# aliddell/acquire-zarr

Hardware: AMD Instinct MI355X
Metric: input GB/s, device-resident multiscale downsample, uint16 frames @1/2/4/8 GPU (higher is better)
Workload: dtype u16

## Files before the change

acquire-zarr_amd/aqz/__init__.py:

```python
from __future__ import annotations

import ctypes as C
import os
import subprocess

import numpy as np

PKG_DIR = os.path.dirname(os.path.dirname(os.path.abspath(__file__)))
LIB_PATH = os.environ.get("AQZ_LIB") or os.path.join(PKG_DIR, "libaqz_gpu.so")

UINT8, UINT16, UINT32, UINT64, INT8, INT16, INT32, INT64, FLOAT32, FLOAT64 = range(10)
DECIMATE, MEAN, MIN, MAX = range(4)
SPACE, CHANNEL, TIME, OTHER = range(4)
MEM_HOST, MEM_DEVICE, MEM_HOST_PINNED = 0, 1, 2

NP_DTYPES = {UINT8: np.uint8, UINT16: np.uint16, UINT32: np.uint32,
             UINT64: np.uint64, INT8: np.int8, INT16: np.int16,
             INT32: np.int32, INT64: np.int64, FLOAT32: np.float32,
             FLOAT64: np.float64}

STATUS = {0: "Success", 1: "InvalidArgument", 2: "Overflow", 3: "InvalidIndex",
          4: "NotYetImplemented", 5: "InternalError", 6: "OutOfMemory",
          9: "InvalidSettings", 12: "WriteOutOfBounds"}

# ... 140 lines not shown
    build_library()
    _preload_hip_runtime()
    L = C.CDLL(LIB_PATH)
    vp, sz, i32, u32, u64 = C.c_void_p, C.c_size_t, C.c_int32, C.c_uint32, C.c_uint64
    D = C.POINTER(Dimension)
    sig = {
        "aqz_version": ([], C.c_char_p),
        "aqz_status_message": ([i32], C.c_char_p),
        "aqz_last_error": ([], C.c_char_p),
        "aqz_device_count": ([C.POINTER(i32)], i32),
        "aqz_dims_create": ([D, sz, i32, C.POINTER(sz), C.POINTER(vp)], i32),
        "aqz_dims_destroy": ([vp], None),
        "aqz_dims_ndims": ([vp], sz),
        "aqz_dims_get": ([vp, sz, D], i32),
        "aqz_dims_tile_group_offset": ([vp, u64], u32),
        "aqz_dims_chunk_internal_offset": ([vp, u64], u64),
        "aqz_dims_chunk_lattice_index": ([vp, u64, u32], u32),
        "aqz_dims_transpose_frame_id": ([vp, u64], u64),
        "aqz_dims_bytes_per_chunk": ([vp], u64),
        "aqz_dims_number_of_chunks_in_memory": ([vp], u32),
        "aqz_dims_frames_per_chunk_layer": ([vp], u64),
        "aqz_dims_shard_index_for_chunk": ([vp, u32], u32),
        "aqz_dims_shard_internal_index": ([vp, u32], u32),
        "aqz_dims_shard_geometry": ([vp, C.POINTER(u32), C.POINTER(u32), C.POINTER(u32)], i32),
        "aqz_dims_skipped_internal_indices": ([vp, u32, u32, C.POINTER(u32), sz,
                                               C.POINTER(sz)], i32),
        "aqz_pyramid_levels": ([D, sz, u32, C.POINTER(u32), D, sz], i32),
        "aqz_dims_split_frame_rows": ([vp, vp, u64, u32, u32, u32, vp, sz, vp, sz], i32),
        "aqz_stage_split_level0_host": ([vp, vp, u64, u64, u32, vp, sz, vp, sz], i32),
        "aqz_stage_split_level0_rows": ([vp, vp, u64, u32, u32, vp, u32, vp, sz, vp, sz], i32),
        "aqz_dims_dim1_banding": ([vp, C.POINTER(i32), C.POINTER(u32), C.POINTER(u64),
                                   C.POINTER(u32)], i32),
        "aqz_downsampling_method_name": ([i32], C.c_char_p),
        "aqz_downsampling_metadata_json": ([i32, C.c_char_p, sz, C.POINTER(sz)], i32),
        "aqz_downsampler_create": ([C.POINTER(ArrayDescC), C.POINTER(vp)], i32),
        "aqz_downsampler_destroy": ([vp], None),
        "aqz_downsampler_n_levels": ([vp], u32),
        "aqz_downsampler_level_dims": ([vp, u32, D, sz, C.POINTER(sz)], i32),
        "aqz_downsampler_add_frame": ([vp, vp, sz, i32], i32),
        "aqz_downsampler_take_frame": ([vp, u32, vp, sz, i32, C.POINTER(sz), C.POINTER(i32)], i32),
        "aqz_downsampler_method_name": ([vp], C.c_char_p),
        "aqz_downsampler_metadata_json": ([vp, C.c_char_p, sz, C.POINTER(sz)], i32),
        "aqz_stage_create": ([C.POINTER(ArrayDescC), C.POINTER(StageOptionsC), C.POINTER(vp)], i32),
        "aqz_stage_create_bench": ([C.POINTER(ArrayDescC), C.POINTER(StageOptionsC),
                                    C.POINTER(StageBenchOptionsC), C.POINTER(vp)], i32),
        "aqz_stage_wait_stream": ([vp, vp], i32),
        "aqz_stage_band_geometry": ([vp, u32, C.POINTER(i32), C.POINTER(u32), C.POINTER(u64),
                                     C.POINTER(u32)], i32),
        "aqz_stage_copy_band_async": ([vp, u32, u64, u32, vp, sz, vp, sz], i32),
        "aqz_stage_memory_usage": ([vp, C.POINTER(MemoryUsageC)], i32),
        "aqz_stage_estimate_memory": ([C.POINTER(ArrayDescC), C.POINTER(StageOptionsC),
                                       C.POINTER(MemoryUsageC)], i32),
        "aqz_stage_estimate_memory_bench": ([C.POINTER(ArrayDescC), C.POINTER(StageOptionsC),
                                             C.POINTER(StageBenchOptionsC),
                                             C.POINTER(MemoryUsageC)], i32),
        "aqz_stage_placement_report": ([vp, C.POINTER(PlacementReportC)], i32),
        "aqz_stage_destroy": ([vp], None),
        "aqz_stage_n_levels": ([vp], u32),
        "aqz_stage_level_dims": ([vp, u32, D, sz, C.POINTER(sz)], i32),
        "aqz_stage_level_layout": ([vp, u32, C.POINTER(LevelLayoutC)], i32),
        "aqz_stage_set_stream": ([vp, vp], i32),
        "aqz_stage_set_tuning": ([vp, u32, u32], i32),
        "aqz_stage_append": ([vp, vp, u64, i32], i32),
        "aqz_stage_synchronize": ([vp], i32),
        "aqz_stage_frames_written": ([vp, u32], u64),
        "aqz_stage_copy_layer": ([vp, u32, u64, vp, sz, vp, sz, i32], i32),
        "aqz_stage_copy_layer_async": ([vp, u32, u64, vp, sz, vp, sz], i32),
        "aqz_stage_frames_consumed": ([vp], u64),
        "aqz_stage_wait_consumed": ([vp, u64], i32),
        "aqz_stage_last_ticket": ([vp], u64),
        "aqz_stage_copies_completed": ([vp], u64),
        "aqz_stage_wait_ticket": ([vp, u64], i32),
        "aqz_stage_wait_copies": ([vp], i32),
        "aqz_host_alloc": ([sz, C.POINTER(vp)], i32),
        "aqz_host_free": ([vp], None),
        "aqz_stage_device_layer": ([vp, u32, u64, C.POINTER(vp), C.POINTER(vp)], i32),
        "aqz_stage_finalize": ([vp], i32),
        "aqz_stage_enable_kernel_timing": ([vp, i32], i32),
        "aqz_stage_kernel_timing": ([vp, C.POINTER(C.c_double), C.POINTER(u64)], i32),
        "aqz_stage_timing_mark": ([vp, i32], i32),
        "aqz_stage_timing_elapsed": ([vp, C.POINTER(C.c_double)], i32),
        "aqz_stage_dominant_kernel": ([vp], C.c_char_p),
        "aqz_stage_zstd_far_ranges": ([vp, u32], u32),
        "aqz_probe_hbm": ([i32, i32, u64, u32, C.POINTER(C.c_double), C.POINTER(u64)], i32),
        "aqz_stage_placement": ([vp, C.POINTER(C.c_double), sz, C.POINTER(sz),
                                 C.POINTER(u32)], i32),
        "aqz_stage_host_affinity": ([vp, C.POINTER(i32), C.POINTER(u32)], i32),
        "aqz_stage_compress_layer": ([vp, u32, u64, C.POINTER(CompressionC)], i32),
        "aqz_stage_compressed_offsets": ([vp, u32, u64, C.POINTER(u64), sz], i32),
        "aqz_stage_copy_compressed_async": ([vp, u32, u64, vp, sz], i32),
        "aqz_compressor_create": ([u64, u32, C.POINTER(CompressionC), C.POINTER(vp)], i32),
        "aqz_compressor_destroy": ([vp], None),
        "aqz_compressor_max_bytes": ([u64, u32], u64),
        "aqz_compressor_scratch_bytes": ([C.POINTER(CompressionC), u64, u32, u32], u64),
        "aqz_compressor_run": ([vp, vp, u64, u32, vp, sz, vp, vp], i32),
        "aqz_compressor_blocksize": ([vp], u32),
        "aqz_decompressor_create": ([u64, u32, C.POINTER(vp)], i32),
        "aqz_decompressor_create_for": ([u64, u32, u32, C.POINTER(vp)], i32),
        "aqz_decompressor_destroy": ([vp], None),
        "aqz_decompressor_scratch_bytes": ([u64, u32], u64),
        "aqz_decompressor_scratch_bytes_for": ([u64, u32, u32], u64),
        "aqz_decompressor_last_run_counts": ([vp, C.POINTER(DecodeCountsC)], i32),
        "aqz_stage_verify_prepare": ([vp, u32], i32),
        "aqz_decompressor_run": ([vp, vp, sz, vp, u32, vp, u64, u64, vp, vp], i32),
        "aqz_stage_verify_layer": ([vp, u32, u64, vp, sz], i32),
        "aqz_stage_verify_result": ([vp, u32, u64, C.POINTER(u32), C.POINTER(u32)], i32),
        "aqz_stage_bench_replace_rings": ([vp, u32], i32),
        "aqz_stage_bench_set_ring_offset": ([vp, u64], i32),
        "aqz_stage_bind_host_thread": ([vp], i32),
        "aqz_stage_import_frames": ([vp, vp, u32, u64, u32, u32], i32),
        "aqz_stage_compression_done": ([vp, u32, u64, C.POINTER(C.c_int32)], i32),
        "aqz_stage_compressed_entries": ([vp, u32, u64, C.POINTER(ChunkEntryC), sz], i32),
        "aqz_stage_shard_geometry": ([vp, u32, C.POINTER(u32), C.POINTER(u32),
                                      C.POINTER(u32)], i32),
        "aqz_shard_table_bytes": ([u32], sz),
        "aqz_shard_table": ([vp, vp, u32, vp, sz], i32),
        "aqz_crc32c": ([vp, sz], u32),
        "aqz_shard_table_parse": ([vp, sz, u32, vp, vp, C.POINTER(i32)], i32),
        "aqz_reader_create": ([C.POINTER(ReaderDescC), C.POINTER(vp)], i32),
        "aqz_reader_destroy": ([vp], None),
        "aqz_reader_device_bytes": ([C.POINTER(ReaderDescC)], u64),
        "aqz_reader_layout": ([vp, C.POINTER(LevelLayoutC)], i32),
        "aqz_reader_load_frames": ([vp, vp, sz, i32, vp, vp, u32, i32, vp], i32),
        "aqz_reader_load_chunks": ([vp, vp, u64, vp, u32, vp], i32),
        "aqz_reader_read_frames": ([vp, u32, u32, vp, u64, vp], i32),
        "aqz_reader_status": ([vp, vp, sz, C.POINTER(u32)], i32),
    }
    for name, (args, res) in sig.items():
        f = getattr(L, name)
        f.argtypes = args
        f.restype = res
    _lib = L
    return L


def _check(status: int, what: str) -> None:
    if status != 0:
        msg = lib().aqz_last_error()
        raise AqzError(status, what + (": " + msg.decode() if msg else ""))


PROBE_READ, PROBE_COPY, PROBE_COPY_THIRD, PROBE_READ_THIRD = 0, 1, 2, 3
PROBE_PLAIN_STORES = 0x100
PROBE_PIECES = 0x200
PROBE_DEEP = 0x400


def probe_hbm(shape: int, nbytes: int = 512 << 20, reps: int = 20, device: int = 0):
    ms, rd = C.c_double(0), C.c_uint64(0)
    _check(lib().aqz_probe_hbm(device, shape, nbytes, reps, C.byref(ms), C.byref(rd)),
           "aqz_probe_hbm")
    return ms.value, rd.value


def device_count() -> int:
    n = C.c_int32(0)
    _check(lib().aqz_device_count(C.byref(n)), "aqz_device_count")
    return n.value


def _dims_c(dims):
    arr = (Dimension * len(dims))()
    for i, d in enumerate(dims):
        arr[i] = Dimension(*d)
    return arr

# ... 51 lines not shown

    def frames_per_chunk_layer(self):
        return lib().aqz_dims_frames_per_chunk_layer(self.h)

    def shard_index_for_chunk(self, c):
        return lib().aqz_dims_shard_index_for_chunk(self.h, c)

    def shard_internal_index(self, c):
        return lib().aqz_dims_shard_internal_index(self.h, c)

    def shard_geometry(self):
        a, b, c = C.c_uint32(), C.c_uint32(), C.c_uint32()
        _check(lib().aqz_dims_shard_geometry(self.h, C.byref(a), C.byref(b), C.byref(c)),
               "aqz_dims_shard_geometry")
        return a.value, b.value, c.value

    def skipped_internal_indices(self, shard, layer):
        n = C.c_size_t(0)
        _check(lib().aqz_dims_skipped_internal_indices(self.h, shard, layer, None, 0,
                                                       C.byref(n)), "skipped_internal")
        out = (C.c_uint32 * max(1, n.value))()
        _check(lib().aqz_dims_skipped_internal_indices(self.h, shard, layer, out, n.value,
                                                       C.byref(n)), "skipped_internal")
        return list(out[:n.value])

    def split_frame_rows(self, frame, frame_id, dst, has_data, row_begin=0, row_end=None,
                         chunk0=0):
        frame = np.ascontiguousarray(frame)
        if row_end is None:
            row_end = frame.shape[-2] if frame.ndim >= 2 else 0
        assert dst.dtype == np.uint8 and has_data.dtype == np.uint8
        _check(lib().aqz_dims_split_frame_rows(self.h, frame.ctypes.data, frame_id, row_begin,
                                               row_end, chunk0, dst.ctypes.data, dst.nbytes,
                                               has_data.ctypes.data, has_data.size),
               "aqz_dims_split_frame_rows")

    def dim1_banding(self):
        a, b, c, d = C.c_int32(), C.c_uint32(), C.c_uint64(), C.c_uint32()
        _check(lib().aqz_dims_dim1_banding(self.h, C.byref(a), C.byref(b), C.byref(c),
                                           C.byref(d)), "aqz_dims_dim1_banding")
        return bool(a.value), b.value, c.value, d.value


def downsampling_method_name(method):
    return lib().aqz_downsampling_method_name(method).decode()


def downsampling_metadata_json(method):
    n = C.c_size_t(0)
    _check(lib().aqz_downsampling_metadata_json(method, None, 0, C.byref(n)), "metadata")
    buf = C.create_string_buffer(n.value + 1)
    _check(lib().aqz_downsampling_metadata_json(method, buf, n.value + 1, C.byref(n)),
           "metadata")
    return buf.value.decode()


def estimate_memory(dims, dtype, method, max_levels=0, layer_slots=0,
                    max_batch_frames=0, storage_order=None, placement_tries=0,
                    level0_split_on_host=False, **bench):
    d, keep = _desc(dims, dtype, method, max_levels, True, storage_order, 0)
    o = StageOptionsC(layer_slots, max_batch_frames, 0, 0, 0, placement_tries,
                      int(bool(level0_split_on_host)))
    m = MemoryUsageC()
    b = _bench_options(bench)
    if b is not None:
        _check(lib().aqz_stage_estimate_memory_bench(C.byref(d), C.byref(o), C.byref(b),
                                                     C.byref(m)),
               "aqz_stage_estimate_memory_bench")
    else:
        _check(lib().aqz_stage_estimate_memory(C.byref(d), C.byref(o), C.byref(m)),
               "aqz_stage_estimate_memory")
    return {"device_bytes": m.device_bytes, "pinned_bytes": m.pinned_bytes}


def compressor_max_bytes(chunk_bytes, n_chunks):
    return lib().aqz_compressor_max_bytes(chunk_bytes, n_chunks)


def compressor_scratch_bytes(codec, chunk_bytes, typesize, n_chunks):
    c = CompressionC(*codec)
    return lib().aqz_compressor_scratch_bytes(C.byref(c), chunk_bytes, typesize, n_chunks)


def pyramid_levels(dims, max_levels=0):
    d = _dims_c(dims)
    n = C.c_uint32(0)
    _check(lib().aqz_pyramid_levels(d, len(dims), max_levels, C.byref(n), None, 0),
           "aqz_pyramid_levels")
    nd = max(3, len(dims))
    out = (Dimension * (n.value * nd))()
    _check(lib().aqz_pyramid_levels(d, len(dims), max_levels, C.byref(n), out,
                                    n.value * nd), "aqz_pyramid_levels")
    return [_tuples(out[l * nd:(l + 1) * nd], nd) for l in range(n.value)]


def _desc(dims, dtype, method, max_levels, multiscale, storage_order, device):
    keep = [_dims_c(dims)]
    order = None
    if storage_order is not None:
        order = (C.c_size_t * len(storage_order))(*storage_order)
        keep.append(order)
    d = ArrayDescC(keep[0], len(dims), dtype, 1 if multiscale else 0, method,
                   max_levels, order, device)
    return d, keep


class HostBuffer:

    def __init__(self, nbytes):
        p = C.c_void_p()
        _check(lib().aqz_host_alloc(nbytes, C.byref(p)), "aqz_host_alloc")
        self.ptr = p.value
        self.nbytes = nbytes
        self.array = np.ctypeslib.as_array((C.c_uint8 * nbytes).from_address(self.ptr))

    def view(self, dtype=np.uint8, shape=None):
        a = self.array.view(dtype)
        return a.reshape(shape) if shape is not None else a

    def close(self):
        if getattr(self, "ptr", None) and _lib is not None:
            self.array = None
            _lib.aqz_host_free(self.ptr)
            self.ptr = None

    def __del__(self):
        self.close()


def _ptr(buf):
    if isinstance(buf, HostBuffer):
        return buf.ptr, MEM_HOST_PINNED
    if isinstance(buf, np.ndarray):
        assert buf.flags.c_contiguous
        return buf.ctypes.data, MEM_HOST
    if hasattr(buf, "data_ptr"):
        assert buf.is_contiguous()
        return buf.data_ptr(), (MEM_DEVICE if buf.is_cuda else MEM_HOST)
    raise TypeError(type(buf))


class Downsampler:

    def __init__(self, dims, dtype, method, max_levels=0, storage_order=None,
                 device=0):
        self.dtype = dtype
        d, self._keep = _desc(dims, dtype, method, max_levels, True,
                              storage_order, device)
        h = C.c_void_p()
        _check(lib().aqz_downsampler_create(C.byref(d), C.byref(h)),
               "aqz_downsampler_create")
        self.h = h

    def __del__(self):
        if getattr(self, "h", None) and _lib is not None:
            _lib.aqz_downsampler_destroy(self.h)
            self.h = None

    def n_levels(self):
        return lib().aqz_downsampler_n_levels(self.h)

    def level_dims(self, level):
        out = (Dimension * 16)()
        n = C.c_size_t(0)
        _check(lib().aqz_downsampler_level_dims(self.h, level, out, 16, C.byref(n)),
               "level_dims")
# ... 143 lines not shown
    def frames_written(self, level):
        return lib().aqz_stage_frames_written(self.h, level)

    def split_level0_host(self, frames_ptr, n_frames, first_frame, dst_ptr, cap, has_ptr,
                          has_cap, chunk0=0):
        _check(lib().aqz_stage_split_level0_host(self.h, frames_ptr, n_frames, first_frame,
                                                 chunk0, dst_ptr, cap, has_ptr, has_cap),
               "split_level0_host")

    def split_level0_rows(self, frame_ptr, frame_id, row_begin, row_end, dst_ptr, cap,
                          has_ptr, has_cap, chunk0=0, frame_copy_ptr=None):
        _check(lib().aqz_stage_split_level0_rows(self.h, frame_ptr, frame_id, row_begin,
                                                 row_end, frame_copy_ptr, chunk0, dst_ptr, cap,
                                                 has_ptr, has_cap), "split_level0_rows")

    def frames_consumed(self):
        return lib().aqz_stage_frames_consumed(self.h)

    def copy_layer(self, level, layer):
        lay = self.layout(level)
        nbytes = lay["bytes_per_chunk"] * lay["chunks_per_layer"]
        out = np.empty(nbytes, dtype=np.uint8)
        flags = np.empty(lay["chunks_per_layer"], dtype=np.uint8)
        _check(lib().aqz_stage_copy_layer(self.h, level, layer, out.ctypes.data,
                                          nbytes, flags.ctypes.data, flags.size,
                                          MEM_HOST), "copy_layer")
        return out, flags

    def device_layer(self, level, layer):
        chunks, flags = C.c_void_p(), C.c_void_p()
        _check(lib().aqz_stage_device_layer(self.h, level, layer, C.byref(chunks),
                                            C.byref(flags)), "device_layer")
        return chunks.value, flags.value, layer // self.layout(level)["layer_slots"] + 1

    def copy_layer_async(self, level, layer, dst_ptr, cap, has_data_ptr=None,
                         has_data_cap=0):
        _check(lib().aqz_stage_copy_layer_async(self.h, level, layer, dst_ptr, cap,
                                                has_data_ptr, has_data_cap),
               "copy_layer_async")

    def wait_consumed(self, frames):
        _check(lib().aqz_stage_wait_consumed(self.h, frames), "wait_consumed")
        self._release_consumed()

    def last_ticket(self):
        return lib().aqz_stage_last_ticket(self.h)

    def copies_completed(self):
        return lib().aqz_stage_copies_completed(self.h)

    def wait_ticket(self, ticket):
        _check(lib().aqz_stage_wait_ticket(self.h, ticket), "wait_ticket")

    def wait_copies(self):
        _check(lib().aqz_stage_wait_copies(self.h), "wait_copies")

    def finalize(self):
        _check(lib().aqz_stage_finalize(self.h), "finalize")
        self._release_consumed()

    def enable_kernel_timing(self, on=True):
        _check(lib().aqz_stage_enable_kernel_timing(self.h, 1 if on else 0), "timing")

    def kernel_timing(self):
        ms = C.c_double(0)
        n = C.c_uint64(0)
        _check(lib().aqz_stage_kernel_timing(self.h, C.byref(ms), C.byref(n)), "timing")
        return ms.value, n.value

    def timing_mark(self, which):
        _check(lib().aqz_stage_timing_mark(self.h, which), "timing_mark")

    def timing_elapsed(self):
        ms = C.c_double(0)
        _check(lib().aqz_stage_timing_elapsed(self.h, C.byref(ms)), "timing_elapsed")
        return ms.value

    def dominant_kernel(self):
        return lib().aqz_stage_dominant_kernel(self.h).decode()

    def zstd_far_ranges(self, level):
        return lib().aqz_stage_zstd_far_ranges(self.h, level)

    def bind_host_thread(self):
        _check(lib().aqz_stage_bind_host_thread(self.h), "bind_host_thread")

    def host_affinity(self):
        node, n = C.c_int32(-1), C.c_uint32(0)
        _check(lib().aqz_stage_host_affinity(self.h, C.byref(node), C.byref(n)),
               "host_affinity")
        return node.value, n.value

    def placement(self):
        r = PlacementReportC()
        _check(lib().aqz_stage_placement_report(self.h, C.byref(r)), "placement_report")
        return {"candidates_ms": [round(r.ms[i], 5) for i in range(min(32, r.n))],
                "kept": r.kept, "kept_ms_final": round(r.kept_ms_final, 5),
                "reps": r.reps, "mode": r.mode,
                "peak_device_bytes": r.peak_device_bytes,
                "probe_bus_gbs": round(r.probe_bus_gbs, 1),
                "expected_ms": round(r.expected_ms, 5), "alg_bytes": r.alg_bytes,
                "accepted": bool(r.accepted),
                "stop": {1: "accepted", 2: "every try ran", 3: "no expectation (probe too small)",
                         4: "out of memory"}.get(r.stop, "no search"),
                "candidates_probe_gbs": [round(r.probe_gbs[i], 1)
                                         for i in range(min(32, r.n))]}

    def compress_layer(self, level, layer, codec=CODEC_BLOSC_LZ4, clevel=5, shuffle=1):
        c = CompressionC(codec, clevel, shuffle)
        _check(lib().aqz_stage_compress_layer(self.h, level, layer, C.byref(c)),
               "compress_layer")

    def compression_done(self, level, layer):
        d = C.c_int32(0)
        _check(lib().aqz_stage_compression_done(self.h, level, layer, C.byref(d)),
               "compression_done")
        return bool(d.value)

    def compressed_offsets(self, level, layer):
        n = self.layout(level)["chunks_per_layer"] + 1
        off = np.empty(n, dtype=np.uint64)
        _check(lib().aqz_stage_compressed_offsets(
            self.h, level, layer, off.ctypes.data_as(C.POINTER(C.c_uint64)), n),
            "compressed_offsets")
        return off

    def copy_compressed_async(self, level, layer, dst_ptr, cap):
        _check(lib().aqz_stage_copy_compressed_async(self.h, level, layer, dst_ptr, cap),
               "copy_compressed_async")

    def compressed_entries(self, level, layer):
        n = self.layout(level)["chunks_per_layer"]
        arr = (ChunkEntryC * n)()
        _check(lib().aqz_stage_compressed_entries(self.h, level, layer, arr, n),
               "compressed_entries")
        return [(e.chunk, e.shard, e.internal, e.offset, e.nbytes) for e in arr]

    def shard_geometry(self, level):
        a, b, c = C.c_uint32(), C.c_uint32(), C.c_uint32()
        _check(lib().aqz_stage_shard_geometry(self.h, level, C.byref(a), C.byref(b),
                                              C.byref(c)), "shard_geometry")
        return a.value, b.value, c.value

    def copy_compressed(self, level, layer):
        off = self.compressed_offsets(level, layer)
        out = np.empty(max(1, int(off[-1])), dtype=np.uint8)
        self.copy_compressed_async(level, layer, out.ctypes.data, out.nbytes)
        self.wait_copies()
        return out[:int(off[-1])], off

    def verify_prepare(self, codecs):
        _check(lib().aqz_stage_verify_prepare(self.h, codecs), "verify_prepare")

    def verify_layer(self, level, layer, frames_ptr=None, frames_bytes=0):
        _check(lib().aqz_stage_verify_layer(self.h, level, layer, frames_ptr, frames_bytes),
               "verify_layer")
        n, first = C.c_uint32(), C.c_uint32()
        _check(lib().aqz_stage_verify_result(self.h, level, layer, C.byref(n),
                                             C.byref(first)), "verify_result")
        return n.value, first.value


class Compressor:

    def __init__(self, chunk_bytes, typesize, codec=CODEC_BLOSC_LZ4, clevel=5, shuffle=1):
        c = CompressionC(codec, clevel, shuffle)
# ... 213 lines not shown
```

acquire-zarr_amd/csrc/aqz_capi.cpp:

```cpp
#include "aqz_gpu.h"
#include "aqz_gpu_bench.h"

#include "aqz_engine.hh"
#include "aqz_reader.hh"

#include <cstring>
#include <new>
#include <string>

using namespace aqz;

struct aqz_dims
{
    std::unique_ptr<ArrayDimensions> ad;
};
struct aqz_downsampler
{
    std::unique_ptr<GpuDownsampler> ds;
    int32_t sticky = AQZ_STATUS_SUCCESS;
};
struct aqz_stage
{
    std::unique_ptr<Stage> st;
    int32_t sticky = AQZ_STATUS_SUCCESS;
// ... 885 lines not shown
{
    return guard_sticky(
      st, [&] { st->st->device_layer(level, layer, chunks, has_data); });
}

aqz_status
aqz_stage_finalize(aqz_stage* st)
{
    return guard_sticky(st, [&] { st->st->finalize(); });
}

aqz_status
aqz_stage_split_level0_host(aqz_stage* st, const void* frames, uint64_t n_frames,
                            uint64_t first_frame, uint32_t chunk0, void* dst, size_t cap,
                            uint8_t* has_data, size_t has_data_cap)
{
    if (!st || !st->st)
        return AQZ_STATUS_INVALID_ARGUMENT;
    return guard([&] {
        st->st->split_level0_host(frames, n_frames, first_frame, chunk0, dst, cap, has_data,
                                  has_data_cap);
    });
}

aqz_status
aqz_stage_split_level0_rows(const aqz_stage* st, const void* frame, uint64_t frame_id,
                            uint32_t row_begin, uint32_t row_end, void* frame_copy,
                            uint32_t chunk0, void* dst, size_t cap, uint8_t* has_data,
                            size_t has_data_cap)
{
    if (!st || !st->st)
        return AQZ_STATUS_INVALID_ARGUMENT;
    return guard([&] {
        st->st->split_level0_rows(frame, frame_id, row_begin, row_end, frame_copy, chunk0, dst,
                                  cap, has_data, has_data_cap);
    });
}

aqz_status
aqz_stage_enable_kernel_timing(aqz_stage* st, int32_t enable)
{
    return guard_sticky(st, [&] { st->st->enable_timing(enable != 0); });
}

aqz_status
aqz_stage_kernel_timing(aqz_stage* st, double* total_ms, uint64_t* launches)
{
    return guard_sticky(st, [&] { st->st->timing(total_ms, launches); });
}

aqz_status
aqz_stage_timing_mark(aqz_stage* st, int32_t which)
{
    return guard_sticky(st, [&] { st->st->mark(which); });
}

aqz_status
aqz_stage_timing_elapsed(aqz_stage* st, double* ms)
{
    return guard_sticky(st, [&] {
        const double v = st->st->marked_ms();
        if (ms)
            *ms = v;
    });
}

const char*
aqz_stage_dominant_kernel(const aqz_stage* st)
{
    return st ? st->st->dominant_kernel() : "";
}

uint32_t
aqz_stage_zstd_far_ranges(const aqz_stage* st, uint32_t level)
{
    try {
        return st && st->st ? st->st->zstd_far_ranges(level) : 0;
    } catch (...) {
        return 0;
    }
}

aqz_status
aqz_stage_host_affinity(const aqz_stage* st, int32_t* numa_node, uint32_t* n_cpus)
{
    if (!st)
        return AQZ_STATUS_INVALID_ARGUMENT;
    if (numa_node)
        *numa_node = st->st->numa_node();
    if (n_cpus)
        *n_cpus = uint32_t(st->st->numa_cpus());
    return AQZ_STATUS_SUCCESS;
}

aqz_status
aqz_stage_placement_report(const aqz_stage* st, aqz_placement_report* out)
{
    if (!st || !out)
        return AQZ_STATUS_INVALID_ARGUMENT;
    const PlacementReport& r = st->st->placement();
    *out = aqz_placement_report{};
    out->n = uint32_t(r.ms.size());
    out->kept = uint32_t(r.kept);
    out->reps = r.reps;
    out->mode = r.mode;
    for (size_t i = 0; i < r.ms.size() && i < 32; ++i)
        out->ms[i] = r.ms[i];
    out->kept_ms_final = r.kept_ms_final;
    out->peak_device_bytes = r.peak_device;
    out->probe_bus_gbs = r.probe_bus_gbs;
    out->expected_ms = r.expected_ms;
    out->alg_bytes = r.alg_bytes;
    out->accepted = r.accepted ? 1u : 0u;
    out->stop = r.stop;
    for (size_t i = 0; i < r.probe_gbs.size() && i < 32; ++i)
        out->probe_gbs[i] = r.probe_gbs[i];
    return AQZ_STATUS_SUCCESS;
}

aqz_status
aqz_stage_placement(const aqz_stage* st, double* ms, size_t cap, size_t* n, uint32_t* kept)
{
    if (!st)
        return AQZ_STATUS_INVALID_ARGUMENT;
    const auto& v = st->st->placement_ms();
    if (n)
        *n = v.size();
    if (kept)
        *kept = uint32_t(st->st->placement_best());
    for (size_t i = 0; ms && i < v.size() && i < cap; ++i)
        ms[i] = v[i];
    return AQZ_STATUS_SUCCESS;
}

}

static Compression
to_compression(const aqz_compression* c)
{
    Compression k;
    k.codec = c->codec;
    k.clevel = c->clevel;
    k.shuffle = c->shuffle;
    return k;
}

aqz_status
aqz_stage_compress_layer(aqz_stage* st, uint32_t level, uint64_t layer,
                         const aqz_compression* comp)
{
    if (!comp)
        return AQZ_STATUS_INVALID_ARGUMENT;
    return guard_sticky(
      st, [&] { st->st->compress_layer(level, layer, to_compression(comp)); });
}

aqz_status
aqz_stage_compressed_offsets(aqz_stage* st, uint32_t level, uint64_t layer,
                             uint64_t* offsets, size_t n)
{
    if (!offsets)
        return AQZ_STATUS_INVALID_ARGUMENT;
    return guard_sticky(
      st, [&] { st->st->compressed_offsets(level, layer, offsets, n); });
}

aqz_status
aqz_stage_copy_compressed_async(aqz_stage* st, uint32_t level, uint64_t layer,
                                void* dst, size_t cap)
{
    if (!dst)
        return AQZ_STATUS_INVALID_ARGUMENT;
    return guard_sticky(
      st, [&] { st->st->copy_compressed_async(level, layer, dst, cap); });
}

aqz_status
aqz_compressor_create(uint64_t chunk_bytes, uint32_t typesize,
                      const aqz_compression* comp, aqz_compressor** out)
{
    if (!comp || !out)
        return AQZ_STATUS_INVALID_ARGUMENT;
    *out = nullptr;
    return guard([&] {
        auto h = std::make_unique<aqz_compressor>();
        h->c = std::make_unique<Compressor>(chunk_bytes, typesize, to_compression(comp));
        *out = h.release();
    });
}

void
aqz_compressor_destroy(aqz_compressor* c)
{
    delete c;
}

uint64_t
aqz_compressor_max_bytes(uint64_t chunk_bytes, uint32_t n_chunks)
{
    return Compressor::max_bytes(chunk_bytes, n_chunks);
}

uint64_t
aqz_compressor_scratch_bytes(const aqz_compression* comp, uint64_t chunk_bytes,
                             uint32_t typesize, uint32_t n_chunks)
{
    if (!comp)
        return 0;
    uint64_t n = 0;
    const aqz_status s = guard([&] {
        const Compression c = to_compression(comp);
        Compressor check(chunk_bytes, typesize, c);
        n = Compressor::scratch_bytes(c, chunk_bytes, typesize, n_chunks);
    });
    return s == AQZ_STATUS_SUCCESS ? n : 0;
}

uint32_t
aqz_compressor_blocksize(const aqz_compressor* c)
{
    return c && c->c ? c->c->blocksize() : 0;
}

aqz_status
aqz_compressor_run(aqz_compressor* c, const void* chunks, uint64_t pitch,
                   uint32_t n_chunks, void* dst, size_t dst_cap, uint64_t* offsets,
                   void* stream)
{
    if (!c || !chunks || !dst || !offsets)
        return AQZ_STATUS_INVALID_ARGUMENT;
    return guard_sticky(c, [&] {
        const uint64_t nb = c->c->chunk_bytes();
        if (pitch < nb)
            throw Error(1, "chunk pitch below the chunk size");
        if (dst_cap < Compressor::max_bytes(nb, n_chunks))
            throw Error(2, "destination below aqz_compressor_max_bytes");
        c->c->run(static_cast<const uint8_t*>(chunks), pitch, n_chunks, nullptr, 0,
                  static_cast<uint8_t*>(dst), offsets, static_cast<hipStream_t>(stream));
    });
}

static_assert(AQZ_DECODE_OK == dec::kOk && AQZ_DECODE_SKIPPED == dec::kSkipped &&
                AQZ_DECODE_BAD_HEADER == dec::kBadHeader &&
                AQZ_DECODE_CORRUPT == dec::kCorrupt &&
                AQZ_DECODE_UNSUPPORTED == dec::kUnsupported,
              "decode status values");

aqz_status
aqz_decompressor_create(uint64_t max_chunk_bytes, uint32_t max_chunks, aqz_decompressor** out)
{
    if (!out)
        return AQZ_STATUS_INVALID_ARGUMENT;
    *out = nullptr;
    return guard([&] {
        auto h = std::make_unique<aqz_decompressor>();
        h->d = std::make_unique<Decompressor>(max_chunk_bytes, max_chunks);
        *out = h.release();
    });
}

static_assert(AQZ_DECODE_CODEC_LZ4 == dec::kFamilyLz4 && AQZ_DECODE_CODEC_ZSTD == dec::kFamilyZstd &&
                AQZ_DECODE_ZSTD_PARALLEL == kDecodeZstdParallel,
              "decode codec bits");

aqz_status
aqz_decompressor_create_for(uint64_t max_chunk_bytes, uint32_t max_chunks, uint32_t codecs,
                            aqz_decompressor** out)
{
    if (!out)
        return AQZ_STATUS_INVALID_ARGUMENT;
    *out = nullptr;
    if (!decode_codecs_valid(codecs))
        return AQZ_STATUS_INVALID_ARGUMENT;
    return guard([&] {
        auto h = std::make_unique<aqz_decompressor>();
        h->d = std::make_unique<Decompressor>(max_chunk_bytes, max_chunks, true, codecs);
        *out = h.release();
    });
}

void
aqz_decompressor_destroy(aqz_decompressor* d)
{
    delete d;
}

uint64_t
aqz_decompressor_scratch_bytes(uint64_t max_chunk_bytes, uint32_t max_chunks)
{
    return Decompressor::scratch_bytes(max_chunk_bytes, max_chunks);
}

uint64_t
aqz_decompressor_scratch_bytes_for(uint64_t max_chunk_bytes, uint32_t max_chunks, uint32_t codecs)
{
    return Decompressor::scratch_bytes(max_chunk_bytes, max_chunks, true, codecs);
}

aqz_status
aqz_decompressor_last_run_counts(aqz_decompressor* d, aqz_decode_counts* out)
// ... 223 lines not shown
```

acquire-zarr_amd/csrc/aqz_codec.hh:

```
#pragma once

#include "aqz_zstd.hh"

#include <hip/hip_runtime.h>

#include <cstdint>

namespace aqz {

constexpr uint32_t kLz4StreamMax = 4096;
constexpr int kLz4HashLog = 10;

struct BloscGeom
{
    uint32_t nbytes;
    uint32_t typesize;
    uint32_t shuffle;
    uint32_t blocksize;
    uint32_t nfull;
    uint32_t left;
    uint32_t ns_full;
    uint32_t spc;
    uint32_t slot;
    uint32_t nblocks;
// ... 79 lines not shown
};

struct ZstdParams
{
    const uint8_t* src;
    uint64_t src_pitch;
    const uint8_t* chunks;
    uint64_t pitch;
    uint32_t n_chunks, nbytes, typesize, shuffle;
    uint32_t blosc;
    uint32_t seg_bytes;
    uint32_t nseg;
    uint32_t bps;
    uint32_t store_only;
    uint32_t match;
    uint32_t match_bits;
    uint32_t phist;
    uint32_t ngrp;
    uint32_t hgrp_log2;
    uint32_t fit;
    uint32_t* far;
    uint32_t far_tb;
    uint32_t far_slices;
    uint32_t far_log;
    uint32_t far_ranges;
    uint32_t far_warm;
    uint32_t dbg;
    const uint32_t* flags;
    uint32_t tag;
    const zstd::SeqTables* seqt;
    uint8_t* lits;
    uint64_t* seqs;
    uint32_t* snseq, *snlit, *stail;
    uint32_t* sval;
    uint32_t* hist;
    uint8_t* bkind;
    uint8_t* bltype;
    uint32_t* bpay;
    uint32_t* bseqb;
    uint32_t* bnlit;
    uint32_t* bpos;
    uint8_t* scratch;
    uint32_t* bnseq;
    ZstdSegTable* tab;
    uint32_t* carrier;
    uint32_t* scount;
    ZstdSeqSeg* sqt;
    uint32_t* scarrier;
    uint32_t* ssize;
    uint8_t* sraw;
    uint32_t* spos;
    uint32_t* fsize;
    uint8_t* mode;
    const uint32_t* order;
    uint64_t* offsets;
    uint64_t* cstart;
    uint8_t* out;
};

constexpr uint32_t kZSub = 4096;
constexpr uint32_t kZSubBlocks = zstd::kBlock / kZSub;
constexpr uint32_t kZSubSeq = 1024;
constexpr uint32_t kZHist1 = 12 * 1024;
constexpr uint32_t kZHist2 = 28 * 1024;
constexpr uint32_t kFarLog = 15;
constexpr uint32_t kFarMin = 5;
constexpr uint32_t kFarWarm = 256;
constexpr uint32_t kZOffMax = (1u << 24) - 4;
inline uint32_t
zstd_far_tag_bits(uint32_t seg_bytes, uint32_t slices, uint32_t far_log = kFarLog)
{
    uint32_t pb = 0, sb = 0;
    while (pb < 32 && (uint64_t(1) << pb) <= seg_bytes)
        ++pb;
    while ((1u << sb) < slices)
        ++sb;
    const uint32_t room = 32 - sb - far_log;
    const uint32_t tb = 32 - pb < room ? 32 - pb : room;
    return tb >= 6 ? tb : 0;
}

hipError_t launch_zstd(const ZstdParams& p, hipStream_t stream);

}
```

acquire-zarr_amd/csrc/aqz_codec.hip:

```cpp
#include "aqz_codec.hh"
#include "aqz_zstd.hh"

namespace aqz {

BloscGeom
make_blosc_geom(uint32_t nbytes, uint32_t typesize, uint32_t shuffle)
{
    BloscGeom g{};
    g.nbytes = nbytes;
    g.typesize = typesize;
    g.shuffle = shuffle;
    uint64_t bs = uint64_t(kLz4StreamMax) * typesize;
    if (bs > nbytes)
        bs = nbytes;
    bs -= bs % typesize;
    if (bs == 0)
        bs = nbytes;
    g.blocksize = uint32_t(bs);
    g.nfull = bs ? nbytes / g.blocksize : 0;
    g.left = bs ? nbytes % g.blocksize : 0;
    g.ns_full = (typesize <= 16 && g.blocksize / typesize >= 128) ? typesize : 1;
    g.spc = g.nfull * g.ns_full + (g.left ? 1u : 0u);
    g.nblocks = g.nfull + (g.left ? 1u : 0u);
    g.slot = g.blocksize / g.ns_full;
// ... 2057 lines not shown
        const uint8_t* scr = p.scratch + uint64_t(g) * zstd::kBlock;
        const uint32_t ns = p.bnseq[g];
        const ZstdSeqSeg& Q = p.sqt[z.seg];
        const bool fitted = ns > 0 && Q.mode == 2;
        const bool scar = fitted && p.scarrier[z.seg] == z.b;
        const uint32_t sd = scar ? Q.desc_n : 0;
        uint8_t* q = d + 3;
        uint32_t lit_bytes = pay;
        if (p.bltype[g] == 2) {
            const ZstdSegTable& T = p.tab[z.grp];
            const bool carry = p.carrier[z.grp] == z.b;
            const uint32_t cs = pay + (carry ? T.tree_n : 0);
            const uint32_t lh = zstd::lit_header_huf_bytes(nl, cs);
            if (t == 0) {
                zstd::write_block_header(d, last, 2, lh + cs + sq + sd);
                zstd::write_lit_header_huf(d + 3, carry ? 2 : 3, nl, cs);
            }
            q += lh;
            if (carry) {
                for (uint32_t i = t; i < T.tree_n; i += 256)
                    q[i] = T.tree[i];
                q += T.tree_n;
            }
        } else {
            const uint32_t lh = zstd::lit_header_raw_bytes(nl);
            if (t == 0) {
                zstd::write_block_header(d, last, 2, lh + nl + sq + sd);
                zstd::write_lit_header_raw(d + 3, 0, nl);
            }
            q += lh;
            lit_bytes = nl;
        }
        if (!fitted) {
            copy_bytes(q, scr, lit_bytes + sq);
        } else {
            const uint32_t kc = ns < 128 ? 1u : ns < 0x7F00 ? 2u : 3u;
            copy_bytes(q, scr, lit_bytes + kc);
            if (t == 0)
                q[lit_bytes + kc] = scar ? uint8_t(2u << 6 | 2u << 4 | 2u << 2)
                                         : uint8_t(3u << 6 | 3u << 4 | 3u << 2);
            uint8_t* qd = q + lit_bytes + kc + 1;
            for (uint32_t i = t; i < sd; i += 256)
                qd[i] = Q.desc[i];
            copy_bytes(qd + sd, scr + lit_bytes + kc + 1, sq - kc - 1);
        }
    }
}

}

hipError_t
launch_shuffle_blocks(const ShuffleParams& p, hipStream_t stream)
{
    if (p.n_chunks == 0 || p.nblocks == 0)
        return hipSuccess;
    if (p.nblocks > 0x7fffffffu || p.n_chunks > 65535u)
        return hipErrorInvalidValue;
    const uint64_t wg = uint64_t(p.nblocks) * p.n_chunks;
    const uint32_t parts = uint32_t(std::min<uint64_t>(16, std::max<uint64_t>(1, (2048 + wg - 1) / wg)));
    hipLaunchKernelGGL(shuffle_blocks, dim3(p.nblocks, p.n_chunks, parts), dim3(256), 0, stream,
                       p);
    return hipGetLastError();
}

hipError_t
launch_blosc_lz4(const BloscParams& p, hipStream_t stream)
{
    if (p.n_chunks == 0)
        return hipSuccess;
    const uint64_t ns = uint64_t(p.n_chunks) * p.g.spc;
    if (ns > 0x7fffffffull || p.g.spc == 0)
        return hipErrorInvalidValue;
    hipLaunchKernelGGL(lz4_streams, dim3(uint32_t(ns)), dim3(64), 0, stream, p);
    hipLaunchKernelGGL(chunk_layout, dim3(p.n_chunks), dim3(256), 0, stream, p);
    hipLaunchKernelGGL(scan_offsets, dim3(1), dim3(256), 0, stream, p.fsize, p.order,
                       p.offsets, p.cstart, p.n_chunks);
    hipLaunchKernelGGL(write_frames, dim3(uint32_t(ns)), dim3(256), 0, stream, p);
    return hipGetLastError();
}

hipError_t
launch_zstd(const ZstdParams& p, hipStream_t stream)
{
    if (p.n_chunks == 0)
        return hipSuccess;
    const uint64_t nseg = uint64_t(p.n_chunks) * p.nseg;
    const uint64_t nblk = nseg * p.bps;
    if (nblk * kZSubBlocks > 0x7fffffffull || p.nseg == 0 || p.bps == 0 ||
        uint64_t(p.bps) * zstd::kBlock < p.seg_bytes)
        return hipErrorInvalidValue;
    if (p.hgrp_log2 > 5 || p.ngrp != ((p.bps + (1u << p.hgrp_log2) - 1) >> p.hgrp_log2))
        return hipErrorInvalidValue;
    if (!p.store_only) {
        hipError_t e = hipMemsetAsync(p.scount, 0, nseg * 192 * 4, stream);
        if (e != hipSuccess)
            return e;
        if (p.match) {
            e = hipMemsetAsync(p.hist, 0, nblk * 256 * 4, stream);
            if (e != hipSuccess)
                return e;
            const dim3 gd(uint32_t(nblk * kZSubBlocks));
            if (p.far) {
                const uint32_t S = p.far_slices;
                if (!(S == 1 || S == 2 || S == 4 || S == 8) || p.far_tb < 6 ||
                    p.far_log < 10 || p.far_log > kFarLog ||
                    p.far_tb + p.far_log + (S == 8 ? 3 : S == 4 ? 2 : S == 2 ? 1 : 0) > 32 ||
                    (reinterpret_cast<uintptr_t>(p.src) & 3u) || (p.src_pitch & 3u) ||
                    (p.seg_bytes & 3u))
                    return hipErrorInvalidValue;
                static const hipError_t attr = hipFuncSetAttribute(
                  reinterpret_cast<const void*>(zstd_far),
                  hipFuncAttributeMaxDynamicSharedMemorySize, int(4u << kFarLog));
                if (attr != hipSuccess)
                    return attr;
                const uint32_t R = p.far_ranges;
                if (!(R == 1 || R == 2 || R == 4 || R == 8))
                    return hipErrorInvalidValue;
                hipLaunchKernelGGL(zstd_far, dim3(uint32_t(nseg * p.far_slices * R)),
                                   dim3(kFarThreads), size_t(4) << p.far_log, stream, p);
            }
            if (p.phist == 0 && !p.far)
                hipLaunchKernelGGL((zstd_parse<0, kLz4HashLog>), gd, dim3(64), 0, stream, p);
            else if (p.phist <= kZHist1 && !p.far)
                hipLaunchKernelGGL((zstd_parse<kZHist1, 13>), gd, dim3(64), 0, stream, p);
            else if (!p.far)
                hipLaunchKernelGGL((zstd_parse<kZHist2, 14>), gd, dim3(64), 0, stream, p);
            else if (p.phist == 0)
                hipLaunchKernelGGL((zstd_parse<0, kLz4HashLog, true>), gd, dim3(64), 0, stream, p);
            else if (p.phist <= kZHist1)
                hipLaunchKernelGGL((zstd_parse<kZHist1, 13, true>), gd, dim3(64), 0, stream, p);
            else
                hipLaunchKernelGGL((zstd_parse<kZHist2, 14, true>), gd, dim3(64), 0, stream, p);
        } else {
            hipLaunchKernelGGL(zstd_hist, dim3(uint32_t(nblk)), dim3(256), 0, stream, p);
        }
        hipLaunchKernelGGL(zstd_table, dim3(uint32_t(nseg * p.ngrp)), dim3(64), 0, stream, p);
        hipLaunchKernelGGL(zstd_encode, dim3(uint32_t(nblk)), dim3(256), 0, stream, p);
        hipLaunchKernelGGL(zstd_seqtab, dim3(uint32_t(nseg)), dim3(64), 0, stream, p);
        if (p.match)
            hipLaunchKernelGGL(zstd_seqenc, dim3(uint32_t(nseg * ((p.bps + 63) / 64))), dim3(64), 0,
                               stream, p);
        hipLaunchKernelGGL(zstd_segment, dim3(uint32_t(nseg)), dim3(64), 0, stream, p);
    }
    hipLaunchKernelGGL(zstd_chunk, dim3(p.n_chunks), dim3(256), 0, stream, p);
    hipLaunchKernelGGL(scan_offsets, dim3(1), dim3(256), 0, stream, p.fsize, p.order,
                       p.offsets, p.cstart, p.n_chunks);
    hipLaunchKernelGGL(zstd_write, dim3(uint32_t(nblk)), dim3(256), 0, stream, p);
    return hipGetLastError();
}

}
```

acquire-zarr_amd/csrc/aqz_engine.cpp:

```cpp
#include <cstdio>
#include "aqz_engine.hh"

#include <hsa/hsa_ext_amd.h>
#include "aqz_zstd.hh"

#include <algorithm>
#include <atomic>
#include <cstdlib>
#include <cstring>
#include <thread>

namespace aqz {


constexpr int kMemDevice = 1;
constexpr int kMemHostPinned = 2;

void
hip_check(hipError_t e, const char* what)
{
    if (e != hipSuccess) {
        (void)hipGetLastError();
        throw Error(e == hipErrorOutOfMemory ? 6 : 5,
                    std::string(what) + ": " + hipGetErrorString(e));
// ... 199 lines not shown
    const uint64_t per = std::max<uint64_t>(1, copy_piece_bytes() / bpc);
    for (uint64_t c = 0; c < n; c += per) {
        const uint64_t m = std::min<uint64_t>(per, n - c);
        if (m > 1)
            hip_check(hipMemcpy2DAsync(static_cast<uint8_t*>(dst) + c * bpc, bpc,
                                       src + c * pitch, pitch, bpc, m, kind, stream),
                      "hipMemcpy2DAsync");
        else
            memcpy_pieces(static_cast<uint8_t*>(dst) + c * bpc, src + c * pitch, bpc,
                          kind, stream);
    }
}

static unsigned
copy_workers()
{
    if (const char* s = std::getenv("AQZ_COPY_THREADS"))
        return unsigned(std::max(0, std::atoi(s)));
    const unsigned hw = std::max(1u, std::thread::hardware_concurrency());
    return std::min(7u, hw / 2);
}

static hipMemcpyKind
kind_from(int src_mem, int dst_mem)
{
    if (src_mem == kMemDevice)
        return dst_mem == kMemDevice ? hipMemcpyDeviceToDevice
                                     : hipMemcpyDeviceToHost;
    return dst_mem == kMemDevice ? hipMemcpyHostToDevice : hipMemcpyHostToHost;
}

static bool
method_valid(int32_t m)
{
    return m >= 0 && m < 4;
}

static bool
pinned_host(const void* p)
{
    hipPointerAttribute_t a{};
    if (hipPointerGetAttributes(&a, p) != hipSuccess) {
        (void)hipGetLastError();
        return false;
    }
    return a.type == hipMemoryTypeHost;
}

static bool
find_hsa_agents(int device, hsa_agent_t* gpu, hsa_agent_t* cpu)
{
    hipDeviceProp_t prop{};
    if (hipGetDeviceProperties(&prop, device) != hipSuccess || hsa_init() != HSA_STATUS_SUCCESS)
        return false;
    struct Find
    {
        uint32_t bdf, domain;
        hsa_agent_t gpu{ 0 }, cpu{ 0 };
    } f{ (uint32_t(prop.pciBusID) << 8) | (uint32_t(prop.pciDeviceID) << 3),
         uint32_t(prop.pciDomainID) };
    auto cb = [](hsa_agent_t a, void* data) -> hsa_status_t {
        auto* f = static_cast<Find*>(data);
        hsa_device_type_t t;
        if (hsa_agent_get_info(a, HSA_AGENT_INFO_DEVICE, &t) != HSA_STATUS_SUCCESS)
            return HSA_STATUS_SUCCESS;
        if (t == HSA_DEVICE_TYPE_CPU && !f->cpu.handle)
            f->cpu = a;
        if (t == HSA_DEVICE_TYPE_GPU) {
            uint32_t bdf = 0, dom = 0;
            hsa_agent_get_info(a, hsa_agent_info_t(HSA_AMD_AGENT_INFO_BDFID), &bdf);
            hsa_agent_get_info(a, hsa_agent_info_t(HSA_AMD_AGENT_INFO_DOMAIN), &dom);
            if ((bdf & ~7u) == f->bdf && dom == f->domain)
                f->gpu = a;
        }
        return HSA_STATUS_SUCCESS;
    };
    if (hsa_iterate_agents(cb, &f) != HSA_STATUS_SUCCESS || !f.gpu.handle || !f.cpu.handle)
        return false;
    *gpu = f.gpu;
    *cpu = f.cpu;
    return true;
}

Stage::Stage(const ArrayDesc& desc, const StageOptions& opt)
  : desc_(desc)
  , opt_(opt)
{
    bpp_ = bytes_of_type(desc.dtype);
    if (desc.multiscale && !method_valid(desc.method))
        throw Error(1, "Invalid downsampling method");
    if (opt_.layer_slots == 0)
        opt_.layer_slots = 2;
    if (opt_.max_batch_frames == 0)
        opt_.max_batch_frames = 64;
    if (opt_.level0_on_host)
        opt_.skip_level0_split = true;

    auto base = std::make_unique<ArrayDimensions>(desc.dims, desc.dtype,
                                                  desc.storage_order);
    if (base->needs_xy_transposition()) {
        if (opt_.level0_on_host)
            throw Error(9, "level0_split_on_host needs storage rows = acquisition rows "
                           "(no XY-transposed storage order)");
        xy_ = true;
        const size_t nd = desc.dims.size();
        acq_rows_ = desc.dims[nd - 2].array_size_px;
        acq_cols_ = desc.dims[nd - 1].array_size_px;
    }
    std::vector<std::vector<Dim>> levels;
    if (desc.multiscale)
        levels = make_pyramid_levels(base->dims(), desc.max_levels,
                                     opt_.force_levels);
    else
        levels = { base->dims() };

    hip_check(hipSetDevice(desc.device), "hipSetDevice");
    hip_check(hipStreamCreateWithFlags(&own_stream_, hipStreamNonBlocking),
              "hipStreamCreate");
    stream_ = own_stream_;
    {
        const char* e = std::getenv("AQZ_NUMA");
        char bus[64] = { 0 };
        if (!(e && std::atoi(e) == 0) &&
            hipDeviceGetPCIBusId(bus, int(sizeof(bus)), desc.device) == hipSuccess)
            numa_cpus_ = numa_cpus_for_pci(bus, &numa_node_);
        (void)hipGetLastError();
    }

    const size_t n = base->ndims();
    const uint32_t B = opt_.max_batch_frames;
    DevBuf spacer;
    if (opt_.ring_spacer)
        spacer.alloc(opt_.ring_spacer, opt_.ring_malloc_flags);
    lv_.resize(levels.size());
    for (size_t k = 0; k < levels.size(); ++k) {
        StageLevel& L = lv_[k];
        L.dims = levels[k];
        if (k == 0)
            L.ad = std::move(base);
        else
            L.ad = std::make_unique<ArrayDimensions>(L.dims, desc.dtype);
        L.W = L.dims[n - 1].array_size_px;
        L.H = L.dims[n - 2].array_size_px;
        L.planes = L.dims[n - 3].array_size_px;
        if (k > 0)
            L.xy_shrinks = L.W < lv_[k - 1].W || L.H < lv_[k - 1].H;
        L.tw = L.dims[n - 1].chunk_size_px;
        L.th = L.dims[n - 2].chunk_size_px;
        L.ntx = parts_along(L.W, L.tw);
        L.nty = parts_along(L.H, L.th);
        L.bpc = L.ad->bytes_per_chunk();
        L.n_chunks = L.ad->number_of_chunks_in_memory();
        const uint64_t F = L.ad->frames_per_chunk_layer();
        if (F == 0 || F > 0x7fffffffull)
            throw Error(9, "unsupported frames per chunk layer");
        L.F = uint32_t(F);
        L.pitch = L.bpc + opt_.chunk_pad;
        L.slot_bytes = L.pitch * L.n_chunks;
        L.layer_bytes = L.bpc * L.n_chunks;
        L.n_slots = std::max<uint32_t>(opt_.layer_slots,
                                       (B - 1 + L.F - 1) / L.F + 1);
        L.slot_layer.assign(L.n_slots, -1);

        L.h_tab_off.resize(L.F);
        L.h_tab_grp.resize(L.F);
        for (uint32_t fl = 0; fl < L.F; ++fl) {
// ... 65 lines not shown
        }
    }
    {
        uint32_t tz = 0;
        while (tz < 6 && ((lv_[0].th >> tz) & 1u) == 0)
            ++tz;
        const uint32_t nf = fused_3d_ ? n_levels() - 1 : n_fused_;
        rh_log2_ = std::max<uint32_t>(std::max<uint32_t>(4, nf), tz);
        if (fused_3d_) {
            const uint32_t RW = uint32_t(512 / bpp_);
            fused_3d_ = lv_[0].W % RW == 0 && (lv_[0].H % (1u << rh_log2_)) == 0 &&
                        lv_[0].th % (1u << rh_log2_) == 0 &&
                        lv_[0].tw % uint32_t(16 / bpp_) == 0 &&
                        (1u << rh_log2_) <= uint32_t(kMaxRegionRows);
        }
    }
    knobs_ = opt_.knobs;
    xcd_rot_ = opt_.xcd_rot;
    nt_mode_ = opt_.nt_mode & 7u;
    if (const uint32_t v = opt_.region_rows_log2) {
        if (v >= std::max<uint32_t>(4, n_fused_) && (1u << v) <= uint32_t(kMaxRegionRows))
            rh_log2_ = v;
    }
    if (xy_ && fused_2d_) {
        const bool tail = n_levels() - 1 > n_fused_;
        xy_direct_ = bpp_ <= 4 && rh_log2_ == 6 && !(knobs_ & 128u) &&
                     (!tail || n_fused_ >= 5) && !(knobs_ & 4096u) &&
                     (uint64_t(acq_cols_) * bpp_) % 16 == 0;
    } else if (xy_ && fused_3d_) {
        xy_direct_ = bpp_ <= 4 && rh_log2_ == 6 && n_levels() - 1 <= 4 &&
                     !(knobs_ & 256u) && !(knobs_ & 4096u) &&
                     (uint64_t(acq_cols_) * bpp_) % 16 == 0;
    }

    const Dim& d0 = lv_[0].dims[0];
    if (d0.array_size_px > 0) {
        max_frames_ = 1;
        for (size_t i = 0; i + 2 < n; ++i)
            max_frames_ *= lv_[0].dims[i].array_size_px;
    }
    if (opt_.z_slab_begin != 0 || opt_.z_slab_end != 0) {
        const uint64_t p0 = lv_[0].planes;
        const uint64_t b0 = opt_.z_slab_begin, e0 = opt_.z_slab_end;
        if (n < 4 || p0 == 0 || b0 >= e0 || e0 > p0)
            throw Error(1, "z slab needs a z dimension and 0 <= begin < end <= planes");
        if (opt_.first_frame % p0 != 0)
            throw Error(1, "with a z slab, first_frame must start a z stack");
        slab_len_ = e0 - b0;
        for (auto& L : lv_) {
            const uint64_t pk = L.planes;
            if ((b0 * pk) % p0 != 0 || (e0 * pk) % p0 != 0)
                throw Error(9, "z slab does not align with the z pyramid");
            slab_skip_.push_back(pk - (e0 - b0) * pk / p0);
        }
        opt_.first_frame += b0;
    }
    if (opt_.first_frame > 0) {
        const uint64_t p0 = std::max<uint32_t>(1, lv_[0].planes);
        for (auto& L : lv_) {
            const uint64_t pk = std::max<uint32_t>(1, L.planes);
            if ((opt_.first_frame * pk) % p0 != 0)
                throw Error(9, "first_frame does not align with the z pyramid");
            L.frames_written = opt_.first_frame * pk / p0;
            L.level_frame_count = uint32_t(L.frames_written);
        }
    }
    pend_.resize(lv_.size());
    for (int j = 0; j < 2; ++j) {
        hip_check(hipEventCreateWithFlags(&h2d_ev_[j], hipEventDisableTiming),
                  "hipEventCreate");
        hip_check(hipEventCreateWithFlags(&consume_ev_[j], hipEventDisableTiming),
                  "hipEventCreate");
    }
    {
        int least = 0, greatest = 0;
        hip_check(hipDeviceGetStreamPriorityRange(&least, &greatest),
                  "hipDeviceGetStreamPriorityRange");
        hip_check(hipStreamCreateWithPriority(&h2d_, hipStreamNonBlocking, greatest),
                  "hipStreamCreate");
        hip_check(hipStreamCreateWithPriority(&d2h_, hipStreamNonBlocking, greatest),
                  "hipStreamCreate");
        for (hipStream_t* cs : { &comp_, &comp_lo_ })
            hip_check(hipStreamCreateWithFlags(cs, hipStreamNonBlocking), "hipStreamCreate");
        hip_check(hipStreamCreateWithPriority(&comp_lo2_, hipStreamNonBlocking, least),
                  "hipStreamCreate");
    }
    if (const char* e = std::getenv("AQZ_D2H_SDMA"); e && std::atoi(e) != 0)
        sdma_d2h_ = find_hsa_agents(desc.device, &hsa_gpu_, &hsa_cpu_);
    for (auto& L : lv_) {
        hip_check(hipEventCreateWithFlags(&L.ops_ev, hipEventDisableTiming),
                  "hipEventCreate");
        if (!L.ring.p)
            continue;
        L.ready_ev.assign(L.n_slots, nullptr);
        L.copy_ev.assign(L.n_slots, nullptr);
        L.copy_pending.assign(L.n_slots, 0);
        for (uint32_t s = 0; s < L.n_slots; ++s) {
            hip_check(hipEventCreateWithFlags(&L.ready_ev[s], hipEventDisableTiming),
                      "hipEventCreate");
            hip_check(hipEventCreateWithFlags(&L.copy_ev[s], hipEventDisableTiming),
                      "hipEventCreate");
        }
        L.flag_bytes.alloc(size_t(L.n_slots) * L.n_chunks);
    }

    calibrate_placement();
    hip_check(hipStreamSynchronize(stream_), "hipStreamSynchronize");
}

void
Stage::place_level(StageLevel& L, uint8_t* at)
{
    if (at)
        L.ring.set_view(at, L.slot_bytes * L.n_slots);
    else
        L.ring.alloc(L.slot_bytes * L.n_slots, opt_.ring_malloc_flags & ~kRingsPlain);
    L.flags.alloc(size_t(L.n_chunks) * L.n_slots * 4);
    hip_check(hipMemsetAsync(L.ring.p, 0, L.ring.n, stream_), "hipMemsetAsync");
    hip_check(hipMemsetAsync(L.flags.p, 0, L.flags.n, stream_), "hipMemsetAsync");
    std::vector<FrameRef> tab(L.period);
    for (uint64_t fid = 0; fid < L.period; ++fid) {
        const uint64_t slot = fid / L.F;
        tab[fid].tiles = L.ring.p + slot * L.slot_bytes + L.h_tab_off[fid % L.F];
        tab[fid].flags = reinterpret_cast<uint32_t*>(L.flags.p) + slot * L.n_chunks +
                         L.h_tab_grp[fid % L.F];
    }
    L.ref_table.alloc(size_t(L.period) * sizeof(FrameRef));
    hip_check(hipMemcpy(L.ref_table.p, tab.data(), size_t(L.period) * sizeof(FrameRef),
                        hipMemcpyHostToDevice),
              "hipMemcpy");
}

void
Stage::calibrate_placement()
{
    const uint32_t tries = opt_.placement_tries;
    const uint32_t reps = std::max<uint32_t>(1, opt_.placement_reps);
    uint64_t ring_bytes = 0, set_bytes = 0;
    std::vector<bool> has_ring(lv_.size());
    for (size_t k = 0; k < lv_.size(); ++k) {
        has_ring[k] = lv_[k].ring.p != nullptr;
        ring_bytes += lv_[k].ring.n;
        set_bytes += lv_[k].ring.n + lv_[k].flags.n + lv_[k].ref_table.n;
    }
    uint32_t n = opt_.max_batch_frames;
    if (fused_3d_ && !fused_2d_)
        n = n / g3d_ * g3d_;
    if (tries <= 1 || n == 0 || !(fused_2d_ || fused_3d_) || (xy_ && !xy_direct_) ||
        ring_bytes < (uint64_t(256) << 20))
        return;
    const bool arena = arena_.p != nullptr;
    if (arena)
        set_bytes = set_bytes - ring_bytes + arena_.physical();
    const uint64_t fb0 = uint64_t(lv_[0].W) * lv_[0].H * bpp_;
    DevBuf src;
    alloc_large(src, size_t(n) * fb0, arena);
    hip_check(hipMemsetAsync(src.p, 0, src.n, stream_), "hipMemsetAsync");
    hip_check(launch_fill_random(src.p, src.n, 0x5eedull, stream_), "fill launch");
    uint64_t live = memory_usage().device + src.n;
    uint64_t peak = live;
    hipEvent_t a = nullptr, b = nullptr;
    hip_check(hipEventCreate(&a), "hipEventCreate");
    hip_check(hipEventCreate(&b), "hipEventCreate");
    std::vector<uint64_t> fw0, lfc0;
    for (const auto& L : lv_) {
        fw0.push_back(L.frames_written);
        lfc0.push_back(L.level_frame_count);
    }
    constexpr uint32_t kWarm = 2;
    std::vector<uint64_t> emitted(lv_.size(), 0);
    auto restore = [&]() {
        for (size_t k = 0; k < lv_.size(); ++k) {
            lv_[k].frames_written = fw0[k];
            lv_[k].level_frame_count = uint32_t(lfc0[k]);
            lv_[k].slot_layer.assign(lv_[k].n_slots, -1);
        }
    };
    auto elapsed = [&]() {
        hip_check(hipEventSynchronize(b), "hipEventSynchronize");
// ... 127 lines not shown
        lv_[k].ring = std::move(best.ring[k]);
        lv_[k].flags = std::move(best.flags[k]);
        lv_[k].ref_table = std::move(best.ref[k]);
    }
    rep.kept_ms_final = measure();
    rep.peak_device = peak;
    placement_ = rep;
    for (auto& L : lv_) {
        if (!L.ring.p)
            continue;
        hip_check(hipMemsetAsync(L.ring.p, 0, L.ring.n, stream_), "hipMemsetAsync");
        hip_check(hipMemsetAsync(L.flags.p, 0, L.flags.n, stream_), "hipMemsetAsync");
    }
    hip_check(hipStreamSynchronize(stream_), "hipStreamSynchronize");
    (void)hipEventDestroy(a);
    (void)hipEventDestroy(b);
}

void
Stage::grant_access(int device)
{
    if (!arena_.p || !arena_.vmm_span)
        return;
    std::lock_guard<std::mutex> lk(access_mu_);
    if (std::find(granted_.begin(), granted_.end(), device) != granted_.end())
        return;
    hipMemAccessDesc acc{};
    acc.location.type = hipMemLocationTypeDevice;
    acc.location.id = device;
    acc.flags = hipMemAccessFlagsProtReadWrite;
    hip_check(hipMemSetAccess(arena_.p, arena_.vmm_span, &acc, 1), "hipMemSetAccess");
    granted_.push_back(device);
}

void
Stage::place_rings_at(uint64_t offset)
{
    uint64_t at = offset;
    for (size_t k = 0; k < lv_.size(); ++k) {
        StageLevel& L = lv_[k];
        if (!(k == 0 && opt_.skip_level0_split)) {
            place_level(L, arena_.p + at);
            at += (L.slot_bytes * L.n_slots + 0xffffull) & ~0xffffull;
        }
    }
}

void
Stage::set_ring_offset(uint64_t offset)
{
    if (!arena_.p)
        throw Error(1, "the stage has no ring arena (bench option ring_arena_bytes)");
    if (offset % 256 || offset + arena_rings_ > arena_.n)
        throw Error(1, "ring offset outside the arena's slack (or not 256-B aligned)");
    hip_check(hipStreamSynchronize(stream_), "hipStreamSynchronize");
    place_rings_at(offset);
    for (auto& L : lv_) {
        L.frames_written = 0;
        L.level_frame_count = 0;
        L.slot_layer.assign(L.n_slots, -1);
    }
    hip_check(hipStreamSynchronize(stream_), "hipStreamSynchronize");
}

void
Stage::replace_rings(uint32_t mask)
{
    synchronize();
    for (size_t k = 0; k < lv_.size() && k < 32; ++k) {
        StageLevel& L = lv_[k];
        if (!((mask >> k) & 1u) || !L.ring.p)
            continue;
        held_.push_back(std::move(L.ring));
        held_.push_back(std::move(L.flags));
        held_.push_back(std::move(L.ref_table));
        place_level(L);
    }
    hip_check(hipStreamSynchronize(stream_), "hipStreamSynchronize");
}

Stage::~Stage()
{
    zpool_.reset();
    for (auto& L : lv_)
        for (auto& v : L.peer_ev)
            for (const auto& e : v)
                (void)hipEventSynchronize(e.get());
    if (stream_)
        (void)hipStreamSynchronize(stream_);
    for (hipStream_t s : { h2d_, comp_, comp_lo_, comp_lo2_, d2h_ })
        if (s) {
            (void)hipStreamSynchronize(s);
            (void)hipStreamDestroy(s);
        }
    for (int j = 0; j < 2; ++j)
        for (hipEvent_t e : { h2d_ev_[j], consume_ev_[j] })
            if (e)
                (void)hipEventDestroy(e);
    for (size_t i = inflight_head_; i < inflight_.size(); ++i)
        if (inflight_[i].first)
            free_ev_.push_back(inflight_[i].first);
    for (const Ticket& t : tickets_) {
        if (t.ev)
            free_ev_.push_back(t.ev);
        if (t.sig.handle) {
            while (hsa_signal_wait_scacquire(t.sig, HSA_SIGNAL_CONDITION_LT, 1, UINT64_MAX,
                                             HSA_WAIT_STATE_BLOCKED) > 0) {
            }
            free_sig_.push_back(t.sig);
        }
    }
    for (hipEvent_t e : free_ev_)
        (void)hipEventDestroy(e);
    for (hsa_signal_t g : free_sig_)
        (void)hsa_signal_destroy(g);
    for (auto& L : lv_) {
        if (L.ops_ev)
            (void)hipEventDestroy(L.ops_ev);
        for (hipEvent_t e : L.ready_ev)
            if (e)
                (void)hipEventDestroy(e);
        for (hipEvent_t e : L.copy_ev)
            if (e)
                (void)hipEventDestroy(e);
        for (hipEvent_t e : L.comp_ev)
            if (e)
                (void)hipEventDestroy(e);
        for (hipEvent_t e : L.cdone_ev)
            if (e)
                (void)hipEventDestroy(e);
        for (hipEvent_t e : L.zin_ev)
            if (e)
                (void)hipEventDestroy(e);
        for (hipEvent_t e : L.verify_ev)
            if (e)
                (void)hipEventDestroy(e);
    }

    for (auto& pr : ev_pairs_) {
        (void)hipEventDestroy(pr.first);
        (void)hipEventDestroy(pr.second);
    }
    for (hipEvent_t e : mark_ev_)
        if (e)
            (void)hipEventDestroy(e);
    if (ext_ev_)
        (void)hipEventDestroy(ext_ev_);
    if (own_stream_)
        (void)hipStreamDestroy(own_stream_);
}

const std::vector<Dim>&
Stage::level_dims(uint32_t level) const
{
    if (level >= lv_.size())
        throw Error(3, "level out of range");
    return lv_[level].dims;
}

LevelLayout
Stage::layout(uint32_t level) const
{
    if (level >= lv_.size())
        throw Error(3, "level out of range");
    const StageLevel& L = lv_[level];
    return LevelLayout{ L.bpc,   L.n_chunks,
                        L.n_slots, L.F,
                        uint64_t(L.W) * L.H * bpp_, L.W,
                        L.H,     L.pitch };
}

void
Stage::set_stream(hipStream_t s)
{
    hip_check(hipStreamSynchronize(stream_), "hipStreamSynchronize");
    stream_ = s ? s : own_stream_;
}

uint64_t
Stage::frames_written(uint32_t level) const
{
    if (level >= lv_.size())
        throw Error(3, "level out of range");
    return lv_[level].frames_written;
}

void
Stage::synchronize()
{
    hip_check(hipStreamSynchronize(h2d_), "hipStreamSynchronize");
    hip_check(hipStreamSynchronize(stream_), "hipStreamSynchronize");
    hip_check(hipStreamSynchronize(comp_), "hipStreamSynchronize");
    hip_check(hipStreamSynchronize(comp_lo_), "hipStreamSynchronize");
    hip_check(hipStreamSynchronize(comp_lo2_), "hipStreamSynchronize");
    hip_check(hipStreamSynchronize(d2h_), "hipStreamSynchronize");
    retire_consumed(true);
}

void
Stage::note_consumed(hipStream_t s, uint64_t frames)
{
    appended_ += frames;
    if (!s) {
        if (inflight_head_ == inflight_.size())
            consumed_ = appended_;
        else
            inflight_.emplace_back(nullptr, appended_);
        return;
    }
    hipEvent_t e;
    if (free_ev_.empty()) {
        hip_check(hipEventCreateWithFlags(&e, hipEventDisableTiming), "hipEventCreate");
    } else {
        e = free_ev_.back();
        free_ev_.pop_back();
    }
    hip_check(hipEventRecord(e, s), "hipEventRecord");
    inflight_.emplace_back(e, appended_);
    retire_consumed(false);
}

void
Stage::retire_consumed(bool wait)
{
    while (inflight_head_ < inflight_.size()) {
        auto& [e, n] = inflight_[inflight_head_];
        if (e) {
            if (wait) {
                hip_check(hipEventSynchronize(e), "hipEventSynchronize");
            } else {
                const hipError_t q = hipEventQuery(e);
                if (q == hipErrorNotReady)
                    break;
                hip_check(q, "hipEventQuery");
            }
            free_ev_.push_back(e);
        }
        consumed_ = n;
        ++inflight_head_;
    }
    if (inflight_head_ == inflight_.size()) {
        inflight_.clear();
        inflight_head_ = 0;
    }
}

uint64_t
Stage::frames_consumed()
{
    retire_consumed(false);
    return consumed_;
}

void
Stage::wait_consumed(uint64_t frames)
{
    if (frames > appended_)
        throw Error(1, "wait_consumed beyond the frames appended");
    while (consumed_ < frames && inflight_head_ < inflight_.size()) {
        auto& [e, n] = inflight_[inflight_head_];
        if (e) {
            hip_check(hipEventSynchronize(e), "hipEventSynchronize");
            free_ev_.push_back(e);
        }
        consumed_ = n;
        ++inflight_head_;
    }
    retire_consumed(false);
}

uint64_t
Stage::issue_ticket()
{
    hipEvent_t e;
    if (free_ev_.empty()) {
        hip_check(hipEventCreateWithFlags(&e, hipEventDisableTiming), "hipEventCreate");
    } else {
        e = free_ev_.back();
        free_ev_.pop_back();
    }
    hip_check(hipEventRecord(e, d2h_), "hipEventRecord");
    tickets_.push_back(Ticket{ e, hsa_signal_t{ 0 } });
    ++tickets_issued_;
    (void)copies_completed();
    return tickets_issued_;
}

uint64_t
Stage::issue_ticket(hsa_signal_t sig)
{
    tickets_.push_back(Ticket{ nullptr, sig });
    ++tickets_issued_;
    (void)copies_completed();
    return tickets_issued_;
}

uint64_t
Stage::copies_completed(bool wait_all, uint64_t until)
{
    while (!tickets_.empty() && tickets_done_ < tickets_issued_) {
        const Ticket t = tickets_.front();
        const bool wait = wait_all || tickets_done_ < until;
        if (t.sig.handle) {
            if (wait) {
                while (hsa_signal_wait_scacquire(t.sig, HSA_SIGNAL_CONDITION_LT, 1, UINT64_MAX,
                                                 HSA_WAIT_STATE_BLOCKED) > 0) {
                }
            } else if (hsa_signal_load_scacquire(t.sig) > 0) {
                break;
            }
            free_sig_.push_back(t.sig);
        } else {
            if (wait) {
                hip_check(hipEventSynchronize(t.ev), "hipEventSynchronize");
            } else {
                const hipError_t q = hipEventQuery(t.ev);
                if (q == hipErrorNotReady)
                    break;
                hip_check(q, "hipEventQuery");
            }
            free_ev_.push_back(t.ev);
        }
        tickets_.pop_front();
        ++tickets_done_;
    }
    return tickets_done_;
}

void
Stage::wait_copies()
{
    hip_check(hipStreamSynchronize(comp_), "hipStreamSynchronize");
    hip_check(hipStreamSynchronize(comp_lo_), "hipStreamSynchronize");
    hip_check(hipStreamSynchronize(comp_lo2_), "hipStreamSynchronize");
    hip_check(hipStreamSynchronize(d2h_), "hipStreamSynchronize");
    (void)copies_completed(true);
}

void
Stage::append(const void* frames, uint64_t n_frames, int mem)
{
    if (n_frames == 0)
        return;
    if (!frames)
        throw Error(1, "null frames");
    finalized_ = false;
    const uint64_t fbytes = uint64_t(lv_[0].W) * lv_[0].H * bpp_;
    uint64_t n_ok = n_frames;
    if (max_frames_ > 0) {
        uint64_t room = max_frames_ - std::min(max_frames_, lv_[0].frames_written);
        if (slab_len_) {
            const uint64_t p0 = lv_[0].planes;
            const uint64_t stack = lv_[0].frames_written / p0;
            const uint64_t stacks = max_frames_ / p0;
            room = stack < stacks ? (stacks - stack) * slab_len_ - slab_done_ : 0;
        }
        n_ok = std::min(n_ok, room);
    }
    const auto* src = static_cast<const uint8_t*>(frames);
    const uint32_t B = opt_.max_batch_frames;
    for (uint64_t done = 0; done < n_ok;) {
        uint32_t b = uint32_t(std::min<uint64_t>(B, n_ok - done));
        if (slab_len_)
            b = uint32_t(std::min<uint64_t>(b, slab_len_ - slab_done_));
        const uint8_t* p = src + done * fbytes;
        if (mem == kMemDevice) {
            run_batch(p, b);
        } else {
            const int j = stage_idx_;
            stage_idx_ ^= 1;
            const size_t nbytes = size_t(b) * fbytes;
            alloc_large(d_stage_[j], size_t(B) * fbytes, opt_.codec.vmm);
            const uint8_t* hsrc = p;
            if (mem != kMemHostPinned) {
                h_stage_[j].alloc(size_t(B) * fbytes);
                hip_check(hipEventSynchronize(h2d_ev_[j]), "hipEventSynchronize");
                if (!pool_)
                    pool_ = std::make_unique<CopyPool>(copy_workers(), numa_cpus_);
                pool_->copy(h_stage_[j].p, p, nbytes);
                hsrc = h_stage_[j].p;
            }
            if (consume_rec_[j])
                hip_check(hipStreamWaitEvent(h2d_, consume_ev_[j], 0),
                          "hipStreamWaitEvent");
            memcpy_pieces(d_stage_[j].p, hsrc, nbytes, hipMemcpyHostToDevice, h2d_);
            hip_check(hipEventRecord(h2d_ev_[j], h2d_), "hipEventRecord");
            if (mem == kMemHostPinned)
                note_consumed(h2d_, b);
            hip_check(hipStreamWaitEvent(stream_, h2d_ev_[j], 0), "hipStreamWaitEvent");
            run_batch(d_stage_[j].p, b);
            hip_check(hipEventRecord(consume_ev_[j], stream_), "hipEventRecord");
            consume_rec_[j] = true;
        }
        if (mem == kMemDevice)
            note_consumed(stream_, b);
        else if (mem != kMemHostPinned)
            note_consumed(nullptr, b);
        done += b;
        if (slab_len_ && (slab_done_ += b) == slab_len_) {
            for (size_t k = 0; k < lv_.size(); ++k) {
                lv_[k].frames_written += slab_skip_[k];
                lv_[k].level_frame_count += uint32_t(slab_skip_[k]);
            }
            slab_done_ = 0;
        }
    }
    if (n_ok < n_frames)
        throw Error(12, "append beyond the array's bounded extent");
}

void
Stage::run_batch(const uint8_t* dsrc, uint32_t n)
{
    uint32_t n3 = 0;
    if (!fused_2d_ && fused_3d_) {
        bool idle = lv_[0].frames_written % g3d_ == 0 &&
                    reinterpret_cast<uintptr_t>(dsrc) % 16 == 0;
// ... 760 lines not shown
}

void
Stage::compressed_entries(uint32_t level, uint64_t layer, ChunkEntry* out, size_t n)
{
    if (level >= lv_.size())
        throw Error(3, "level out of range");
    StageLevel& L = lv_[level];
    const uint32_t slot = L.n_slots ? uint32_t(layer % L.n_slots) : 0;
    if (L.comp_layer.empty() || L.comp_layer[slot] != int64_t(layer))
        throw Error(3, "layer was not compressed (or its slot was reused)");
    if (n < L.n_chunks)
        throw Error(2, "entries too small");
    const uint64_t* off;
    if (L.comp_host[slot]) {
        HostLayerJob& j = *L.zjob[slot];
        j.wait();
        if (j.status)
            throw Error(j.status, "zstd compression failed");
        off = j.offsets.data();
    } else {
        hip_check(hipEventSynchronize(L.comp_ev[slot]), "hipEventSynchronize");
        off = reinterpret_cast<const uint64_t*>(L.h_coffsets[slot].p);
    }
    const uint32_t cl = uint32_t(layer % L.layers_per_shard);
    for (uint32_t i = 0; i < L.n_chunks; ++i) {
        const uint32_t c = L.h_order[i];
        out[i] = ChunkEntry{ c, L.h_shard[c], L.h_internal0[c] + cl * L.internal_stride, 0,
                             off[i], off[i + 1] - off[i] };
    }
}

void
Stage::shard_geometry(uint32_t level, uint32_t* chunks_per_shard, uint32_t* n_shards,
                      uint32_t* layers_per_shard) const
{
    if (level >= lv_.size())
        throw Error(3, "level out of range");
    const StageLevel& L = lv_[level];
    if (chunks_per_shard)
        *chunks_per_shard = L.chunks_per_shard;
    if (n_shards)
        *n_shards = L.n_shards;
    if (layers_per_shard)
        *layers_per_shard = L.layers_per_shard;
}

Compressor::Compressor(uint64_t chunk_bytes, uint32_t typesize, const Compression& c,
                       const CodecTuning& tune)
  : c_(c)
  , tune_(tune)
  , nbytes_(chunk_bytes)
  , typesize_(typesize)
{
    if (c.codec < 1 || c.codec > 3)
        throw Error(4, "unknown codec");
    if (c.codec != 3 && (c.shuffle < 0 || c.shuffle > 2 || c.clevel < 0 || c.clevel > 9))
        throw Error(1, "invalid compression settings");
    if (c.codec == 3 && (c.clevel < 0 || c.clevel > 22 || c.shuffle != 0))
        throw Error(1, "invalid zstd settings: level 0-22 and no shuffle");
    if (chunk_bytes == 0 || chunk_bytes > 0x7fffffefull || typesize == 0 ||
        typesize > 255)
        throw Error(1, "chunk size outside the blosc1 limits");
    if (c.codec == 1)
        g_ = make_blosc_geom(uint32_t(chunk_bytes), typesize, uint32_t(c.shuffle));
    store_only_ = c.codec != 3 && c.clevel == 0;
}

constexpr uint64_t kFarRangeCus = 256;

uint32_t
zstd_far_slices(const Compression& c, uint32_t typesize)
{
    (void)typesize;
    if (c.codec == 3) {
        const int zl = c.clevel == 0 ? 3 : c.clevel;
        return zl >= 7 ? 8u : zl >= 3 ? 4u : 0u;
    }
    if (c.codec == 2 && c.shuffle == 2 && c.clevel >= 2)
        return 1u;
    return 0u;
}

uint64_t
Compressor::scratch_bytes(const Compression& c, uint64_t chunk_bytes, uint32_t typesize,
                          uint32_t n_chunks)
{
    const uint64_t n = n_chunks;
    const bool store_only = c.codec != 3 && c.clevel == 0;
    uint64_t b = n * 4 + n + n * 8;
    if (c.codec == 1) {
        const BloscGeom g = make_blosc_geom(uint32_t(chunk_bytes), typesize, uint32_t(c.shuffle));
        const uint64_t ns = n * g.spc;
        return b + (store_only ? 1 : ns * g.slot) + ns * 8;
    }
    uint64_t seg = chunk_bytes, nseg1 = 1;
    if (c.codec == 2) {
        const ZstdBloscGeom g = make_zstd_blosc_geom(uint32_t(chunk_bytes), typesize);
        seg = g.blocksize;
        nseg1 = g.nblocks;
    }
    const uint64_t nseg = n * nseg1, bps = (seg + zstd::kBlock - 1) / zstd::kBlock;
    const uint32_t gl =
      zstd_huf_group_log2(c.codec == 2 ? uint32_t(c.shuffle) : 0u, typesize, uint32_t(seg),
                          c.clevel);
    const uint64_t nblk = nseg * bps, ngrp = nseg * ((bps + (1u << gl) - 1) >> gl);
    b += nseg * 4;
    if (c.codec == 2 && !store_only && (c.shuffle == 2 || (c.shuffle == 1 && typesize > 1)))
        b += n * chunk_bytes;
    if (store_only)
        return b;
    if (zstd_far_slices(c, typesize))
        b += nseg * seg * 4;
    const uint64_t nu = nblk * kZSubBlocks;
    b += nu * kZSub + nu * kZSubSeq * 8 + 4 * nu * 4;
    b += nblk * (1 + 4 + 4 + 4 + 256 * 4 + 1 + 4 + 4 + zstd::kBlock);
    b += nseg * (192 * 4 + sizeof(ZstdSeqSeg) + 4 + 1 + 4);
    b += ngrp * (sizeof(ZstdSegTable) + 4) + sizeof(zstd::SeqTables);
    return b;
}

void
Compressor::run(const uint8_t* chunks, uint64_t pitch, uint32_t n_chunks,
                const uint32_t* flags, uint32_t tag, uint8_t* out, uint64_t* offsets,
                hipStream_t stream, const uint32_t* order)
{
    if (c_.codec != 1) {
        run_zstd(chunks, pitch, n_chunks, flags, tag, out, offsets, stream, order);
        return;
    }
    const uint64_t ns = uint64_t(n_chunks) * g_.spc;
    alloc_large(scratch_, store_only_ ? 1 : ns * g_.slot, tune_.vmm);
    ssize_.alloc(ns * 4);
    spos_.alloc(ns * 4);
    fsize_.alloc(size_t(n_chunks) * 4);
    mode_.alloc(n_chunks);
    cstart_.alloc(size_t(n_chunks) * 8);
    BloscParams p{};
    p.g = g_;
    p.chunks = chunks;
    p.pitch = pitch;
    p.n_chunks = n_chunks;
    p.flags = flags;
    p.tag = tag;
    p.scratch = scratch_.p;
    p.ssize = reinterpret_cast<uint32_t*>(ssize_.p);
    p.spos = reinterpret_cast<uint32_t*>(spos_.p);
    p.fsize = reinterpret_cast<uint32_t*>(fsize_.p);
    p.mode = mode_.p;
    p.offsets = offsets;
    p.cstart = reinterpret_cast<uint64_t*>(cstart_.p);
    p.order = order;
    p.out = out;
    p.store_only = store_only_ ? 1 : 0;
    hip_check(launch_blosc_lz4(p, stream), "blosc-lz4 launch");
}

void
Compressor::run_zstd(const uint8_t* chunks, uint64_t pitch, uint32_t n_chunks,
                     const uint32_t* flags, uint32_t tag, uint8_t* out, uint64_t* offsets,
                     hipStream_t stream, const uint32_t* order)
{
    const bool blosc = c_.codec == 2;
    ZstdParams p{};
    p.chunks = chunks;
    p.pitch = pitch;
    p.n_chunks = n_chunks;
    p.nbytes = uint32_t(nbytes_);
    p.typesize = typesize_;
    p.shuffle = blosc ? uint32_t(c_.shuffle) : 0;
    p.blosc = blosc ? 1 : 0;
    p.store_only = store_only_ ? 1 : 0;
    p.flags = flags;
    p.tag = tag;
    if (blosc) {
        const ZstdBloscGeom g = make_zstd_blosc_geom(uint32_t(nbytes_), typesize_);
        p.seg_bytes = g.blocksize;
        p.nseg = g.nblocks;
    } else {
        p.seg_bytes = uint32_t(nbytes_);
        p.nseg = 1;
    }
    p.bps = (p.seg_bytes + zstd::kBlock - 1) / zstd::kBlock;
    p.hgrp_log2 = zstd_huf_group_log2(p.shuffle, typesize_, p.seg_bytes, c_.clevel);
    p.ngrp = (p.bps + (1u << p.hgrp_log2) - 1) >> p.hgrp_log2;
    p.phist = tune_.phist;
    p.match_bits = uint32_t(blosc ? zstd::kMatchBits : zstd::kMatchBitsFitted);
    p.fit = tune_.fit;
    p.src = chunks;
    p.src_pitch = pitch;
    p.dbg = tune_.parse & 15u;
    const bool shuffle = blosc && !store_only_ &&
                         (c_.shuffle == 2 || (c_.shuffle == 1 && typesize_ > 1));
    if (shuffle && n_chunks > 65535u)
        throw Error(1, "blosc-zstd with a shuffle takes at most 65535 chunks per run");
    if (shuffle) {
        alloc_large(zin_, size_t(n_chunks) * nbytes_, tune_.vmm);
        ShuffleParams sp{ chunks, pitch, n_chunks, flags, tag, p.nbytes, typesize_,
                          uint32_t(c_.shuffle), p.seg_bytes, p.nseg, zin_.p };
        hip_check(launch_shuffle_blocks(sp, stream), "shuffle launch");
        p.src = zin_.p;
        p.src_pitch = nbytes_;
    }
    const uint64_t nseg = uint64_t(n_chunks) * p.nseg, nblk = nseg * p.bps;
    p.match = tune_.match ? 1 : 0;
    if (!store_only_) {
        if (!seqt_.p) {
            zstd::SeqTables t;
            if (!zstd::build_seq_tables(t))
                throw Error(10, "zstd sequence tables");
            seqt_.alloc(sizeof(t));
            hip_check(hipMemcpy(seqt_.p, &t, sizeof(t), hipMemcpyHostToDevice), "hipMemcpy");
        }
        p.far_slices = zstd_far_slices(c_, typesize_);
        p.far_log = blosc ? 13u : kFarLog;
        p.far_tb = p.far_slices ? zstd_far_tag_bits(p.seg_bytes, p.far_slices, p.far_log) : 0;
        bool far = p.match && p.far_tb != 0 && (reinterpret_cast<uintptr_t>(p.src) & 3u) == 0 &&
                   (p.src_pitch & 3u) == 0 && (p.seg_bytes & 3u) == 0;
        far = far && tune_.far != 0;
        if (far) {
            alloc_large(far_, nseg * p.seg_bytes * 4, tune_.vmm);
            p.far = reinterpret_cast<uint32_t*>(far_.p);
            p.phist = 0;
            const uint64_t wgs = nseg * p.far_slices;
            const uint64_t steps = (uint64_t(p.seg_bytes) + kZSub - 1) / kZSub;
            const uint64_t cus = kFarRangeCus;
            const uint64_t warm = std::max<uint64_t>(kFarWarm, (2 * plane_bytes_ + kZSub - 1) / kZSub);
            p.far_warm = uint32_t(std::min<uint64_t>(warm, steps));
            p.far_ranges = 1;
            while (tune_.ranges && p.far_ranges < 8 && wgs * p.far_ranges * 2 <= cus &&
                   steps / (2u * p.far_ranges) >= warm)
                p.far_ranges *= 2;
        }
        far_ranges_ = far ? p.far_ranges : 0;
        if (p.match) {
            const uint64_t nu = nblk * kZSubBlocks;
            alloc_large(lits_, nu * kZSub, tune_.vmm);
            alloc_large(seqs_, nu * kZSubSeq * 8, tune_.vmm);
            snseq_.alloc(nu * 4);
            snlit_.alloc(nu * 4);
            stail_.alloc(nu * 4);
            sval_.alloc(nu * 4);
        }
        const uint64_t ngrp = nseg * p.ngrp;
        bltype_.alloc(nblk);
        bseqb_.alloc(nblk * 4);
        bnlit_.alloc(nblk * 4);
        bnseq_.alloc(nblk * 4);
        hist_.alloc(nblk * 256 * 4);
        scount_.alloc(nseg * 192 * 4);
        sqt_.alloc(nseg * sizeof(ZstdSeqSeg));
        scarrier_.alloc(nseg * 4);
        bkind_.alloc(nblk);
        bpay_.alloc(nblk * 4);
        bpos_.alloc(nblk * 4);
        alloc_large(scratch_, nblk * zstd::kBlock, tune_.vmm);
        tab_.alloc(ngrp * sizeof(ZstdSegTable));
        carrier_.alloc(ngrp * 4);
        sraw_.alloc(nseg);
        ssize_.alloc(nseg * 4);
    }
    spos_.alloc(nseg * 4);
    fsize_.alloc(size_t(n_chunks) * 4);
    mode_.alloc(n_chunks);
    cstart_.alloc(size_t(n_chunks) * 8);
    p.seqt = reinterpret_cast<const zstd::SeqTables*>(seqt_.p);
    p.lits = lits_.p;
    p.seqs = reinterpret_cast<uint64_t*>(seqs_.p);
    p.snseq = reinterpret_cast<uint32_t*>(snseq_.p);
    p.snlit = reinterpret_cast<uint32_t*>(snlit_.p);
    p.stail = reinterpret_cast<uint32_t*>(stail_.p);
    p.sval = reinterpret_cast<uint32_t*>(sval_.p);
    p.bltype = bltype_.p;
    p.bseqb = reinterpret_cast<uint32_t*>(bseqb_.p);
    p.bnlit = reinterpret_cast<uint32_t*>(bnlit_.p);
    p.hist = reinterpret_cast<uint32_t*>(hist_.p);
    p.bnseq = reinterpret_cast<uint32_t*>(bnseq_.p);
    p.scount = reinterpret_cast<uint32_t*>(scount_.p);
    p.sqt = reinterpret_cast<ZstdSeqSeg*>(sqt_.p);
    p.scarrier = reinterpret_cast<uint32_t*>(scarrier_.p);
    p.bkind = bkind_.p;
    p.bpay = reinterpret_cast<uint32_t*>(bpay_.p);
    p.bpos = reinterpret_cast<uint32_t*>(bpos_.p);
    p.scratch = scratch_.p;
    p.tab = reinterpret_cast<ZstdSegTable*>(tab_.p);
    p.carrier = reinterpret_cast<uint32_t*>(carrier_.p);
    p.ssize = reinterpret_cast<uint32_t*>(ssize_.p);
    p.sraw = sraw_.p;
    p.spos = reinterpret_cast<uint32_t*>(spos_.p);
    p.fsize = reinterpret_cast<uint32_t*>(fsize_.p);
    p.mode = mode_.p;
    p.order = order;
    p.offsets = offsets;
    p.cstart = reinterpret_cast<uint64_t*>(cstart_.p);
    p.out = out;
    hip_check(launch_zstd(p, stream), "zstd launch");
}

void
Stage::ensure_comp_slots(StageLevel& L)
{
    if (!L.cframes.empty())
        return;
    L.cframes.resize(L.n_slots);
    L.coffsets.resize(L.n_slots);
    L.h_coffsets.resize(L.n_slots);
    L.comp_ev.assign(L.n_slots, nullptr);
    L.cdone_ev.assign(L.n_slots, nullptr);
    L.cdone_pending.assign(L.n_slots, 0);
    L.cdone_ticket.assign(L.n_slots, 0);
    L.comp_layer.assign(L.n_slots, -1);
    L.comp_codec.assign(L.n_slots, 0);
    L.h_zin.resize(L.n_slots);
    L.h_zhas.resize(L.n_slots);
    L.zin_ev.assign(L.n_slots, nullptr);
    L.zjob.resize(L.n_slots);
    L.comp_host.assign(L.n_slots, 0);
    for (uint32_t s = 0; s < L.n_slots; ++s) {
        hip_check(hipEventCreateWithFlags(&L.comp_ev[s], hipEventDisableTiming),
                  "hipEventCreate");
        hip_check(hipEventCreateWithFlags(&L.cdone_ev[s], hipEventDisableTiming),
                  "hipEventCreate");
        hip_check(hipEventCreateWithFlags(&L.zin_ev[s], hipEventDisableTiming),
                  "hipEventCreate");
    }
}

static bool
zstd_on_host()
{
    const char* s = std::getenv("AQZ_ZSTD_HOST");
    return s && std::atoi(s) != 0;
}

static unsigned
zstd_workers()
{
    if (const char* s = std::getenv("AQZ_ZSTD_THREADS"))
        return unsigned(std::max(1, std::atoi(s)));
    const unsigned hw = std::max(1u, std::thread::hardware_concurrency());
    return std::min(16u, std::max(1u, hw - 1));
}

void
Stage::compress_layer_host(StageLevel& L, uint32_t slot, uint64_t layer,
                           const Compression& c)
{
    const hipStream_t cs = comp_stream(L);
    const ZstdLib& z = ZstdLib::get();
    if (!z.ok)
        throw Error(4, "libzstd.so.1 is not available: no zstd codecs");
    if (c.codec == 2 && (c.shuffle < 0 || c.shuffle > 2 || c.clevel < 0 || c.clevel > 9))
        throw Error(1, "invalid blosc compression settings");
    if (c.codec == 3 && (c.clevel < -131072 || c.clevel > z.max_clevel()))
        throw Error(1, "invalid zstd level");
    if (L.bpc > 0x7fffffefull)
        throw Error(1, "chunk size outside the blosc1 limits");
    ensure_comp_slots(L);
    if (!zpool_)
        zpool_ = std::make_unique<TaskPool>(zstd_workers(), numa_cpus_);
    if (L.zjob[slot])
        L.zjob[slot]->wait();
    else
        L.zjob[slot] = std::make_shared<HostLayerJob>();
    if (L.cdone_ticket[slot]) {
        (void)copies_completed(false, L.cdone_ticket[slot]);
        L.cdone_ticket[slot] = 0;
    }
    if (L.cdone_pending[slot]) {
        hip_check(hipStreamWaitEvent(cs, L.cdone_ev[slot], 0), "hipStreamWaitEvent");
        L.cdone_pending[slot] = 0;
    }
    L.h_zin[slot].alloc(L.layer_bytes);
    L.h_zhas[slot].alloc(L.n_chunks);
    hip_check(hipEventRecord(L.ready_ev[slot], stream_), "hipEventRecord");
    hip_check(hipStreamWaitEvent(cs, L.ready_ev[slot], 0), "hipStreamWaitEvent");
    const uint8_t* chunks = L.ring.p + slot * L.slot_bytes;
    const auto* flags = reinterpret_cast<const uint32_t*>(L.flags.p) + size_t(slot) * L.n_chunks;
    const uint32_t tag = uint32_t(layer / L.n_slots + 1);
    const bool shuffle = c.codec == 2 && (c.shuffle == 2 || (c.shuffle == 1 && bpp_ > 1));
    if (shuffle) {
        const ZstdBloscGeom g = make_zstd_blosc_geom(uint32_t(L.bpc), uint32_t(bpp_));
        L.d_zshuf.alloc(L.layer_bytes);
        ShuffleParams sp{ chunks, L.pitch, L.n_chunks, flags, tag, uint32_t(L.bpc),
                          uint32_t(bpp_), uint32_t(c.shuffle), g.blocksize, g.nblocks,
                          L.d_zshuf.p };
        hip_check(launch_shuffle_blocks(sp, cs), "shuffle launch");
        memcpy_pieces(L.h_zin[slot].p, L.d_zshuf.p, L.layer_bytes, hipMemcpyDeviceToHost,
                      cs);
    } else {
        copy_chunks(L.h_zin[slot].p, chunks, L.bpc, L.pitch, L.n_chunks,
                    hipMemcpyDeviceToHost, cs);
    }
    uint8_t* fb = L.flag_bytes.p + size_t(slot) * L.n_chunks;
    hip_check(launch_flags_to_bytes(flags, fb, L.n_chunks, tag, cs), "flags launch");
    hip_check(hipMemcpyAsync(L.h_zhas[slot].p, fb, L.n_chunks, hipMemcpyDeviceToHost, cs),
              "hipMemcpyAsync");
    hip_check(hipEventRecord(L.zin_ev[slot], cs), "hipEventRecord");
    hip_check(hipEventRecord(L.copy_ev[slot], cs), "hipEventRecord");
    L.copy_pending[slot] = 1;

    HostLayerJob& j = *L.zjob[slot];
    j.codec = c.codec;
    j.clevel = c.clevel;
    j.shuffle = c.codec == 2 ? c.shuffle : 0;
    j.typesize = uint32_t(bpp_);
    j.bpc = L.bpc;
    j.n_chunks = L.n_chunks;
    j.chunks = L.h_zin[slot].p;
    j.has_data = L.h_zhas[slot].p;
    j.order = L.h_order;
    const ZstdBloscGeom g = make_zstd_blosc_geom(uint32_t(L.bpc), uint32_t(bpp_));
    j.frame_cap = std::max<uint64_t>(z.compress_bound(L.bpc),
                                     L.bpc + 16 + 8ull * g.nblocks + 64);
    j.tmp.resize(size_t(j.frame_cap) * L.n_chunks);
    host_zstd_compress(*zpool_, L.zjob[slot],
                       [ev = L.zin_ev[slot]] { (void)hipEventSynchronize(ev); });
    L.comp_layer[slot] = int64_t(layer);
    L.comp_codec[slot] = c.codec;
    L.comp_host[slot] = 1;
}

void
Stage::compress_layer(uint32_t level, uint64_t layer, const Compression& c)
{
    if (level >= lv_.size())
        throw Error(3, "level out of range");
    StageLevel& L = lv_[level];
    const hipStream_t cs = comp_stream(L);
    if (!L.ring.p)
        throw Error(1, "level 0 is not split on the device by this stage");
    const uint32_t slot = uint32_t(layer % L.n_slots);
    if (L.slot_layer[slot] != int64_t(layer))
        throw Error(3, "chunk layer not resident");
    if ((c.codec == 2 || c.codec == 3) && zstd_on_host()) {
        compress_layer_host(L, slot, layer, c);
        return;
    }
    if (!L.comp || L.comp_cfg.codec != c.codec || L.comp_cfg.clevel != c.clevel ||
        L.comp_cfg.shuffle != c.shuffle) {
        hip_check(hipStreamSynchronize(cs), "hipStreamSynchronize");
        hip_check(hipStreamSynchronize(d2h_), "hipStreamSynchronize");
        L.comp = std::make_unique<Compressor>(L.bpc, uint32_t(bpp_), c, opt_.codec);
        L.comp->set_plane_bytes(uint64_t(L.tw) * L.th * bpp_);
        L.comp_cfg = c;
    }
    ensure_comp_slots(L);
    if (L.zjob[slot])
        L.zjob[slot]->wait();
    L.comp_host[slot] = 0;
    if (L.cdone_ticket[slot]) {
        (void)copies_completed(false, L.cdone_ticket[slot]);
        L.cdone_ticket[slot] = 0;
    }
    if (L.cdone_pending[slot]) {
        hip_check(hipStreamWaitEvent(cs, L.cdone_ev[slot], 0), "hipStreamWaitEvent");
        L.cdone_pending[slot] = 0;
    }
    const uint64_t cap = Compressor::max_bytes(L.bpc, L.n_chunks);
    if (L.cframes[slot].n < cap)
        hip_check(hipStreamSynchronize(cs), "hipStreamSynchronize");
    alloc_large(L.cframes[slot], cap, opt_.codec.vmm);
    L.coffsets[slot].alloc((size_t(L.n_chunks) + 1) * 8);
    L.h_coffsets[slot].alloc((size_t(L.n_chunks) + 1) * 8);
    hip_check(hipEventRecord(L.ready_ev[slot], stream_), "hipEventRecord");
    hip_check(hipStreamWaitEvent(cs, L.ready_ev[slot], 0), "hipStreamWaitEvent");
    L.comp->run(L.ring.p + slot * L.slot_bytes, L.pitch, L.n_chunks,
                reinterpret_cast<const uint32_t*>(L.flags.p) + size_t(slot) * L.n_chunks,
                uint32_t(layer / L.n_slots + 1), L.cframes[slot].p,
                reinterpret_cast<uint64_t*>(L.coffsets[slot].p), cs,
                reinterpret_cast<const uint32_t*>(L.shard_order.p));
    hip_check(hipMemcpyAsync(L.h_coffsets[slot].p, L.coffsets[slot].p,
                             (size_t(L.n_chunks) + 1) * 8, hipMemcpyDeviceToHost, cs),
              "hipMemcpyAsync");
    hip_check(hipEventRecord(L.comp_ev[slot], cs), "hipEventRecord");
    hip_check(hipEventRecord(L.copy_ev[slot], cs), "hipEventRecord");
    L.copy_pending[slot] = 1;
    L.comp_layer[slot] = int64_t(layer);
    L.comp_codec[slot] = c.codec;
}

Decompressor::Decompressor(uint64_t max_chunk_bytes, uint32_t max_chunks, bool big_blocks,
                           uint32_t codecs)
  : max_chunk_bytes_(max_chunk_bytes)
  , max_chunks_(max_chunks)
  , codecs_(codecs)
{
    if (max_chunk_bytes == 0 || max_chunk_bytes > 0x7fffffefull || max_chunks == 0)
        throw Error(1, "chunk size outside the blosc1 limits, or no chunks");
    if (!decode_codecs_valid(codecs))
        throw Error(1, "codecs: AQZ_DECODE_CODEC_LZ4 | AQZ_DECODE_CODEC_ZSTD, "
                       "AQZ_DECODE_ZSTD_PARALLEL only with the latter alone");
    const bool zstd = codecs & dec::kFamilyZstd;
    if (big_blocks || zstd) {
        scratch_pitch_ = (max_chunk_bytes + 15) & ~uint64_t(15);
        scratch_.alloc(scratch_pitch_ * max_chunks);
    }
    if (zstd) {
        zpasses_ = zstd_decode_passes(max_chunk_bytes);
        zlit_pitch_ = zstd_decode_lit_pitch(max_chunk_bytes);
        zlit_.alloc(zlit_pitch_ * zpasses_ * max_chunks);
    }
    if (codecs & kDecodeZstdParallel) {
        zpar_.alloc(zstd_parallel_bytes(max_chunk_bytes, max_chunks));
        hip_check(hipMemset(zpar_.p, 0, 16), "hipMemset");
    }
}

bool
decode_codecs_valid(uint32_t codecs)
{
    const uint32_t fam = codecs & (dec::kFamilyLz4 | dec::kFamilyZstd);
    if (fam == 0 || (codecs & ~(dec::kFamilyLz4 | dec::kFamilyZstd | kDecodeZstdParallel)))
        return false;
    return !(codecs & kDecodeZstdParallel) || codecs == (dec::kFamilyZstd | kDecodeZstdParallel);
}

uint64_t
Decompressor::scratch_bytes(uint64_t max_chunk_bytes, uint32_t max_chunks, bool big_blocks,
                            uint32_t codecs)
{
    if (max_chunk_bytes == 0 || max_chunk_bytes > 0x7fffffefull || !decode_codecs_valid(codecs))
        return 0;
    const bool zstd = codecs & dec::kFamilyZstd;
    uint64_t n = 0;
    if (big_blocks || zstd)
        n += ((max_chunk_bytes + 15) & ~uint64_t(15)) * max_chunks;
    if (zstd)
        n += zstd_decode_lit_pitch(max_chunk_bytes) * zstd_decode_passes(max_chunk_bytes) *
             max_chunks;
    if (codecs & kDecodeZstdParallel)
        n += zstd_parallel_bytes(max_chunk_bytes, max_chunks);
    return n;
}

void
Decompressor::run(const uint8_t* frames, uint64_t frames_bytes, const uint64_t* offsets,
                  uint32_t n_chunks, uint8_t* dst, uint64_t pitch, uint64_t chunk_bytes,
                  uint32_t* status, hipStream_t stream, const uint32_t* order, uint32_t* bad)
{
    if (chunk_bytes == 0 || chunk_bytes > max_chunk_bytes_)
        throw Error(1, "chunk size above the decompressor's max_chunk_bytes");
    if (n_chunks > max_chunks_)
        throw Error(1, "more frames than the decompressor's max_chunks");
    if (pitch < chunk_bytes)
        throw Error(1, "chunk pitch below the chunk size");
    DecodeParams p{};
    p.frames = frames;
    p.frames_bytes = frames_bytes;
    p.offsets = offsets;
    p.n_chunks = n_chunks;
    p.dst = dst;
    p.pitch = pitch;
    p.chunk_bytes = chunk_bytes;
// ... 225 lines not shown
        hsa_signal_t sig{ 0 };
        if (free_sig_.empty()) {
            if (hsa_signal_create(1, 0, nullptr, &sig) != HSA_STATUS_SUCCESS)
                throw Error(5, "hsa_signal_create failed");
        } else {
            sig = free_sig_.back();
            free_sig_.pop_back();
            hsa_signal_store_screlease(sig, 1);
        }
        if (total == 0) {
            hsa_signal_store_screlease(sig, 0);
        } else if (hsa_amd_memory_async_copy(dst, hsa_cpu_, L.cframes[slot].p, hsa_gpu_, total,
                                             0, nullptr, sig) != HSA_STATUS_SUCCESS) {
            free_sig_.push_back(sig);
            throw Error(5, "hsa_amd_memory_async_copy failed");
        }
        last_ticket_ = issue_ticket(sig);
        L.cdone_ticket[slot] = last_ticket_;
        return;
    }
    memcpy_pieces(dst, L.cframes[slot].p, total, hipMemcpyDefault, d2h_);
    hip_check(hipEventRecord(L.copy_ev[slot], d2h_), "hipEventRecord");
    hip_check(hipEventRecord(L.cdone_ev[slot], d2h_), "hipEventRecord");
    L.copy_pending[slot] = 1;
    L.cdone_pending[slot] = 1;
    last_ticket_ = issue_ticket();
}

void
Stage::import_frames(Stage* src, uint32_t level, uint64_t layer, uint32_t first,
                     uint32_t count)
{
    if (level >= lv_.size())
        throw Error(3, "level out of range");
    StageLevel& L = lv_[level];
    if (!L.ring.p)
        throw Error(1, "level 0 is not split on the device by this stage");
    if (uint64_t(first) + count > L.F)
        throw Error(3, "frames outside the chunk layer");
    StageLevel* S = nullptr;
    if (src) {
        if (src->lv_.size() != lv_.size())
            throw Error(1, "stages of different pyramids");
        S = &src->lv_[level];
        if (S->bpc != L.bpc || S->n_chunks != L.n_chunks || S->F != L.F ||
            S->n_slots != L.n_slots || S->pitch != L.pitch || !S->ring.p)
            throw Error(1, "stages of different chunk geometry");
        if (S->slot_layer[layer % S->n_slots] != int64_t(layer))
            throw Error(3, "source chunk layer not resident");
        if (src->desc_.device != desc_.device) {
            const hipError_t e = hipDeviceEnablePeerAccess(src->desc_.device, 0);
            if (e != hipSuccess && e != hipErrorPeerAccessAlreadyEnabled)
                hip_check(e, "hipDeviceEnablePeerAccess");
            (void)hipGetLastError();
            src->grant_access(desc_.device);
        }
    }
    if (count == 0)
        return;
    const uint32_t slot = uint32_t(layer % L.n_slots);
    if (L.slot_layer[slot] != int64_t(layer))
        enter_layer(L, layer);
    if (src) {
        hip_check(hipEventRecord(S->ready_ev[slot], src->stream_), "hipEventRecord");
        hip_check(hipStreamWaitEvent(stream_, S->ready_ev[slot], 0), "hipStreamWaitEvent");
    }
    const uint32_t tile_bytes = L.th * L.tw * uint32_t(bpp_);
    hip_check(launch_import_frames(
                L.ring.p + slot * L.slot_bytes, S ? S->ring.p + slot * S->slot_bytes : nullptr,
                reinterpret_cast<const uint64_t*>(L.tab_off.p),
                reinterpret_cast<const uint32_t*>(L.tab_grp.p), first, count, L.ntx * L.nty,
                L.pitch, tile_bytes,
                reinterpret_cast<uint32_t*>(L.flags.p) + size_t(slot) * L.n_chunks,
                S ? reinterpret_cast<const uint32_t*>(S->flags.p) + size_t(slot) * S->n_chunks
                  : nullptr,
                uint32_t(layer / L.n_slots + 1), stream_),
              "import launch");
    if (src) {
        hipEvent_t e = nullptr;
        hip_check(hipEventCreateWithFlags(&e, hipEventDisableTiming), "hipEventCreate");
        std::shared_ptr<ihipEvent_t> ev(e, [](hipEvent_t x) { (void)hipEventDestroy(x); });
        hip_check(hipEventRecord(e, stream_), "hipEventRecord");
        std::lock_guard<std::mutex> lk(src->access_mu_);
        if (S->peer_ev.empty())
            S->peer_ev.resize(S->n_slots);
        S->peer_ev[slot].push_back(std::move(ev));
    }
}

void
Stage::finalize()
{
    for (auto& L : lv_) {
        if (!L.ring.p)
            continue;
        const uint64_t fw = L.frames_written;
        if (fw % L.F == 0 || L.slot_layer[(fw / L.F) % L.n_slots] != int64_t(fw / L.F))
            continue;
        const uint64_t end = (fw / L.F + 1) * L.F;
        for (uint64_t fid = fw; fid < end; ++fid) {
            uint64_t off;
            uint32_t fo;
            tile_addr(L, fid, &off, &fo, nullptr);
            hip_check(launch_zero_frame_tiles(L.ring.p + off, L.pitch,
                                              L.ntx * L.nty,
                                              uint32_t(uint64_t(L.tw) * L.th * bpp_),
                                              stream_),
                      "zero launch");
        }
    }
    finalized_ = true;
    synchronize();
}

static unsigned
split_workers()
{
    if (const char* s = std::getenv("AQZ_SPLIT_THREADS"))
        return unsigned(std::max(0, std::atoi(s)));
    const unsigned hw = std::max(1u, std::thread::hardware_concurrency());
    return std::min(15u, hw / 2);
}

void
Stage::split_level0_rows(const void* frame, uint64_t frame_id, uint32_t row_begin,
                         uint32_t row_end, void* frame_copy, uint32_t chunk0, void* dst,
                         size_t cap, uint8_t* has_data, size_t has_data_cap) const
{
    const StageLevel& L = lv_[0];
    if (!frame || !dst || !has_data)
        throw Error(1, "null frame, destination or has_data");
    const uint64_t n = std::min<uint64_t>(cap / L.bpc, has_data_cap);
    if (n == 0 || chunk0 >= L.n_chunks)
        throw Error(1, "destination holds no chunk of the layer");
    split_rows(split_geom(*L.ad, frame_id), static_cast<const uint8_t*>(frame), row_begin,
               row_end, static_cast<uint8_t*>(dst), chunk0,
               uint32_t(std::min<uint64_t>(n, L.n_chunks - chunk0)), has_data,
               static_cast<uint8_t*>(frame_copy));
}

void
Stage::split_level0_host(const void* frames, uint64_t n, uint64_t first, uint32_t chunk0,
                         void* dst, size_t cap, uint8_t* has_data, size_t has_data_cap)
{
    if (n == 0)
        return;
    if (!frames)
        throw Error(1, "null frames");
    const StageLevel& L = lv_[0];
    if (first / L.F != (first + n - 1) / L.F)
        throw Error(1, "the frames span two chunk layers");
    const uint64_t fbytes = uint64_t(L.W) * L.H * bpp_;
    constexpr uint32_t kRows = 64;
    const uint32_t per_frame = parts_along(L.H, kRows);
    if (!split_pool_)
        split_pool_ = std::make_unique<SplitPool>(split_workers(), numa_cpus_);
    const auto* src = static_cast<const uint8_t*>(frames);
    split_pool_->run(size_t(n) * per_frame, [&](size_t i) {
        const uint64_t f = i / per_frame;
        const uint32_t r0 = uint32_t(i % per_frame) * kRows;
        split_level0_rows(src + f * fbytes, first + f, r0, std::min(L.H, r0 + kRows), nullptr,
                          chunk0, dst, cap, has_data, has_data_cap);
    });
}

void
Stage::enable_timing(bool on)
{
// ... 283 lines not shown
```

acquire-zarr_amd/csrc/aqz_engine.hh:

```
#pragma once

#include "aqz_codec.hh"
#include "aqz_decode.hh"
#include "aqz_copy.hh"
#include "aqz_geometry.hh"
#include "aqz_hostsplit.hh"
#include "aqz_hostzstd.hh"
#include "aqz_params.hh"

#include <hip/hip_runtime.h>
#include <hsa/hsa.h>

#include <deque>
#include <memory>
#include <mutex>
#include <string>
#include <vector>

namespace aqz {

hipError_t launch_fused_pyramid(int dtype, int method, const FusedParams& p,
                                hipStream_t stream);
hipError_t launch_level(int dtype, int method, const LevelParams& p,
                        hipStream_t stream);
// ... 13 lines not shown
hipError_t launch_zero_frame_tiles(uint8_t* fb, uint64_t bpc,
                                   uint32_t n_tiles, uint32_t tile_bytes,
                                   hipStream_t stream);
constexpr int kPlacementProbeVariants = 3;
uint64_t probe_copy_third_read_bytes(uint64_t src_bytes, uint64_t dst_bytes);
hipError_t launch_probe_copy_third(const uint8_t* src, uint8_t* dst, uint64_t read_bytes,
                                   hipStream_t stream, int variant, bool third_only = false);

void hip_check(hipError_t e, const char* what);

struct DevBuf
{
    uint8_t* p = nullptr;
    size_t n = 0;
    bool view = false;
    std::vector<hipMemGenericAllocationHandle_t> vmm;
    size_t vmm_span = 0;
    size_t vmm_piece = 0;
    size_t vmm_mapped = 0;
    static constexpr unsigned kVmm = 0x100u;
    size_t physical() const { return vmm_span ? vmm_span : n; }
    DevBuf() = default;
    explicit DevBuf(size_t bytes) { alloc(bytes); }
    ~DevBuf();
    DevBuf(const DevBuf&) = delete;
    DevBuf& operator=(const DevBuf&) = delete;
    DevBuf(DevBuf&& o) noexcept;
    DevBuf& operator=(DevBuf&& o) noexcept;
    void alloc(size_t bytes, unsigned flags = 0);
    void set_view(uint8_t* q, size_t bytes);
    void release();
};

struct PinnedBuf
{
    uint8_t* p = nullptr;
    size_t n = 0;
    PinnedBuf() = default;
    ~PinnedBuf();
    PinnedBuf(const PinnedBuf&) = delete;
    PinnedBuf& operator=(const PinnedBuf&) = delete;
    PinnedBuf(PinnedBuf&& o) noexcept
      : p(o.p)
      , n(o.n)
    {
        o.p = nullptr;
        o.n = 0;
    }
    void alloc(size_t bytes);
};

struct Compression
{
    int32_t codec = 0;
    int32_t clevel = 1;
    int32_t shuffle = 1;
};

struct CodecTuning
{
    uint32_t match = 1;
    uint32_t far = 1;
    uint32_t fit = 1;
    uint32_t phist = 0;
    uint32_t parse = 0;
    uint32_t vmm = 0;
    uint32_t ranges = 1;
};

uint32_t zstd_far_slices(const Compression& c, uint32_t typesize);

class Compressor
{
  public:
    Compressor(uint64_t chunk_bytes, uint32_t typesize, const Compression& c,
               const CodecTuning& tune = CodecTuning{});
    static uint64_t max_bytes(uint64_t chunk_bytes, uint32_t n_chunks)
    {
        return uint64_t(n_chunks) *
               (chunk_bytes + 32 + 3 * (chunk_bytes / zstd::kBlock + 1));
    }
    void run(const uint8_t* chunks, uint64_t pitch, uint32_t n_chunks,
             const uint32_t* flags, uint32_t tag, uint8_t* out, uint64_t* offsets,
             hipStream_t stream, const uint32_t* order = nullptr);
    const BloscGeom& geom() const { return g_; }
    void set_plane_bytes(uint64_t b) { plane_bytes_ = b; }
    uint64_t chunk_bytes() const { return nbytes_; }
    uint32_t far_ranges() const { return far_ranges_; }
    uint32_t blocksize() const
    {
        if (c_.codec == 1)
            return g_.blocksize;
        if (c_.codec == 2)
            return make_zstd_blosc_geom(uint32_t(nbytes_), typesize_).blocksize;
        return 0;
    }
    static uint64_t scratch_bytes(const Compression& c, uint64_t chunk_bytes,
                                  uint32_t typesize, uint32_t n_chunks);
    uint64_t device_bytes() const
    {
        uint64_t n = scratch_.n + ssize_.n + spos_.n + fsize_.n + mode_.n + cstart_.n;
        for (const DevBuf* b : { &zin_, &hist_, &scount_, &bkind_, &bpay_, &bpos_, &tab_, &carrier_,
                                 &sraw_, &lits_, &seqs_, &snseq_, &snlit_, &stail_, &bltype_,
                                 &bnseq_, &sqt_, &scarrier_, &sval_,
                                 &bseqb_, &bnlit_, &seqt_, &far_ })
            n += b->n;
        return n;
    }

  private:
    void run_zstd(const uint8_t* chunks, uint64_t pitch, uint32_t n_chunks,
                  const uint32_t* flags, uint32_t tag, uint8_t* out, uint64_t* offsets,
                  hipStream_t stream, const uint32_t* order);
    Compression c_;
    CodecTuning tune_;
    uint64_t nbytes_ = 0;
    uint64_t plane_bytes_ = 0;
    uint32_t far_ranges_ = 0;
    uint32_t typesize_ = 1;
    BloscGeom g_{};
    bool store_only_;
    DevBuf scratch_, ssize_, spos_, fsize_, mode_, cstart_;
    DevBuf zin_, hist_, scount_, bkind_, bpay_, bpos_, tab_, carrier_, sraw_;
    DevBuf bnseq_, sqt_, scarrier_, sval_;
    DevBuf lits_, seqs_, snseq_, snlit_, stail_, bltype_, bseqb_, bnlit_, seqt_, far_;
};

constexpr uint32_t kDecodeZstdParallel = 4;
bool decode_codecs_valid(uint32_t codecs);

class Decompressor
{
  public:
    Decompressor(uint64_t max_chunk_bytes, uint32_t max_chunks, bool big_blocks = true,
                 uint32_t codecs = dec::kFamilyLz4);
    static uint64_t scratch_bytes(uint64_t max_chunk_bytes, uint32_t max_chunks,
                                  bool big_blocks = true, uint32_t codecs = dec::kFamilyLz4);
    void run(const uint8_t* frames, uint64_t frames_bytes, const uint64_t* offsets,
             uint32_t n_chunks, uint8_t* dst, uint64_t pitch, uint64_t chunk_bytes,
             uint32_t* status, hipStream_t stream, const uint32_t* order = nullptr,
             uint32_t* bad = nullptr);
    uint64_t device_bytes() const { return scratch_.n + zlit_.n + zpar_.n; }
    uint32_t codecs() const { return codecs_; }
    void last_run_counts(uint32_t (&counts)[4]);

  private:
    uint64_t max_chunk_bytes_;
    uint32_t max_chunks_;
    uint32_t codecs_;
    uint64_t scratch_pitch_ = 0;
    uint64_t zlit_pitch_ = 0;
    uint32_t zpasses_ = 0;
    DevBuf scratch_, zlit_;
    DevBuf zpar_;
    hipStream_t last_stream_ = nullptr;
};

struct ArrayDesc
{
    std::vector<Dim> dims;
    int32_t dtype = 0;
    bool multiscale = true;
    int32_t method = 0;
    uint32_t max_levels = 0;
    std::vector<size_t> storage_order;
    int32_t device = 0;
};

constexpr uint32_t kRingsPlain = 0x10000u;

struct StageOptions
{
    uint32_t layer_slots = 2;
    uint32_t max_batch_frames = 64;
    uint32_t force_levels = 0;
    bool skip_level0_split = false;
    bool level0_on_host = false;
    uint64_t first_frame = 0;
    uint32_t z_slab_begin = 0, z_slab_end = 0;
    uint32_t placement_tries = 0;
    uint32_t placement_reps = 10;
    bool placement_never_accept = false;
    uint32_t knobs = 0;
    uint32_t nt_mode = 7;
    uint32_t xcd_rot = 0;
    uint32_t region_rows_log2 = 0;
    uint64_t chunk_pad = 0;
    uint32_t ring_malloc_flags = 0;
    uint64_t ring_spacer = 0;
    uint64_t ring_arena = 0;
    CodecTuning codec;
};

struct PlacementReport
{
    std::vector<double> ms;
// ... 19 lines not shown
    uint32_t layer_slots;
    uint64_t frames_per_layer;
    uint64_t frame_bytes;
    uint32_t width, height;
    uint64_t chunk_pitch;
};

struct StageLevel
{
    std::vector<Dim> dims;
    std::unique_ptr<ArrayDimensions> ad;
    uint32_t W = 0, H = 0, planes = 0;
    bool xy_shrinks = false;
    uint64_t bpc = 0;
    uint64_t pitch = 0;
    uint64_t slot_bytes = 0;
    uint64_t layer_bytes = 0;
    uint32_t n_chunks = 0, n_slots = 0, F = 0;
    uint32_t tw = 0, th = 0, ntx = 0, nty = 0;
    DevBuf ring, flags, tab_off, tab_grp, ref_table;
    uint32_t period = 0;
    std::vector<uint64_t> h_tab_off;
    std::vector<uint32_t> h_tab_grp;
    std::vector<int64_t> slot_layer;
    uint64_t frames_written = 0;
    uint32_t level_frame_count = 0;
    DevBuf scratch;
    DevBuf partial[2];
    int carried = -1;
    DevBuf d_ops;
    PinnedBuf h_ops;
    hipEvent_t ops_ev = nullptr;
    std::vector<hipEvent_t> ready_ev, copy_ev;
    std::vector<uint8_t> copy_pending;
    std::vector<std::vector<std::shared_ptr<ihipEvent_t>>> peer_ev;
    DevBuf flag_bytes;
    std::unique_ptr<Compressor> comp;
    Compression comp_cfg;
    std::vector<DevBuf> cframes, coffsets;
    std::vector<PinnedBuf> h_coffsets;
    std::vector<hipEvent_t> comp_ev;
    std::vector<hipEvent_t> cdone_ev;
    std::vector<uint8_t> cdone_pending;
    std::vector<uint64_t> cdone_ticket;
    std::vector<int64_t> comp_layer;
    std::vector<int32_t> comp_codec;
    std::unique_ptr<Decompressor> dec;
    std::unique_ptr<Decompressor> zdec;
    DevBuf voffsets;
    std::vector<DevBuf> vwords;
    std::vector<PinnedBuf> h_vwords;
    std::vector<hipEvent_t> verify_ev;
    std::vector<uint8_t> verify_pending;
    std::vector<int64_t> verify_layer;
    std::vector<PinnedBuf> h_zin, h_zhas;
    std::vector<hipEvent_t> zin_ev;
    std::vector<std::shared_ptr<HostLayerJob>> zjob;
    std::vector<uint8_t> comp_host;
    DevBuf d_zshuf;
    DevBuf shard_order;
    std::vector<uint32_t> h_order, h_shard, h_internal0;
    uint32_t chunks_per_shard = 0, n_shards = 0, layers_per_shard = 1;
    uint32_t internal_stride = 0;
};

struct Footprint
{
    uint64_t device = 0, pinned = 0;
};

struct ChunkEntry
{
    uint32_t chunk, shard, internal, reserved;
    uint64_t offset, nbytes;
};

uint32_t crc32c(const uint8_t* p, size_t n);
void shard_table(const uint64_t* offsets, const uint64_t* extents, uint32_t n,
                 uint8_t* out);

bool shard_major_order(const ArrayDimensions& ad, std::vector<uint32_t>& order,
                       std::vector<uint32_t>& shard, std::vector<uint32_t>& internal0);

class Stage
{
  public:
    Stage(const ArrayDesc& desc, const StageOptions& opt);
    ~Stage();

    uint32_t n_levels() const { return uint32_t(lv_.size()); }
    const std::vector<Dim>& level_dims(uint32_t level) const;
    LevelLayout layout(uint32_t level) const;
    void set_stream(hipStream_t s);
    void wait_stream(hipStream_t s);
    void set_tuning(uint32_t knobs, uint32_t nt) { knobs_ = knobs; nt_mode_ = nt & 7u; }
    void replace_rings(uint32_t mask);
    void set_ring_offset(uint64_t offset);
    void append(const void* frames, uint64_t n_frames, int mem);
    void synchronize();
    uint64_t frames_written(uint32_t level) const;
    uint64_t frames_consumed();
    void wait_consumed(uint64_t frames);
    uint64_t last_ticket() const { return last_ticket_; }
    uint64_t copies_completed(bool wait_all = false, uint64_t until = 0);
    void copy_layer(uint32_t level, uint64_t layer, void* dst, size_t cap,
                    uint8_t* has_data, size_t has_data_cap, int mem);
    void device_layer(uint32_t level, uint64_t layer, void** chunks,
                      uint32_t** flags);
    void copy_layer_async(uint32_t level, uint64_t layer, void* dst, size_t cap,
                          uint8_t* has_data, size_t has_data_cap);
    void wait_copies();
    void band_geometry(uint32_t level, int32_t* supported, uint32_t* n_bands,
                       uint64_t* frames_per_band, uint32_t* chunks_per_band) const;
    void copy_band_async(uint32_t level, uint64_t layer, uint32_t band, void* dst,
                         size_t cap, uint8_t* has_data, size_t has_data_cap);
    Footprint memory_usage() const;
    static Footprint estimate_memory(const ArrayDesc& desc, const StageOptions& opt);
    void compress_layer(uint32_t level, uint64_t layer, const Compression& c);
    void compressed_offsets(uint32_t level, uint64_t layer, uint64_t* offsets,
                            size_t n);
    bool compression_done(uint32_t level, uint64_t layer);
    void copy_compressed_async(uint32_t level, uint64_t layer, void* dst, size_t cap);
    void compressed_entries(uint32_t level, uint64_t layer, ChunkEntry* out, size_t n);
    void shard_geometry(uint32_t level, uint32_t* chunks_per_shard, uint32_t* n_shards,
                        uint32_t* layers_per_shard) const;
    void verify_layer(uint32_t level, uint64_t layer, const void* frames, size_t frames_bytes);
    void verify_prepare(uint32_t codecs);
    void verify_result(uint32_t level, uint64_t layer, uint32_t* n_bad, uint32_t* first_bad);
    void finalize();
    void split_level0_host(const void* frames, uint64_t n, uint64_t first, uint32_t chunk0,
                           void* dst, size_t cap, uint8_t* has_data, size_t has_data_cap);
    void split_level0_rows(const void* frame, uint64_t frame_id, uint32_t row_begin,
                           uint32_t row_end, void* frame_copy, uint32_t chunk0, void* dst,
                           size_t cap, uint8_t* has_data, size_t has_data_cap) const;
    void import_frames(Stage* src, uint32_t level, uint64_t layer, uint32_t first,
                       uint32_t count);
    int device() const { return desc_.device; }
    void enable_timing(bool on);
    void timing(double* total_ms, uint64_t* launches);
    void mark(int which);
    double marked_ms();
    const char* dominant_kernel() const;
    uint32_t zstd_far_ranges(uint32_t level) const
    {
        if (level >= lv_.size())
            throw Error(3, "level out of range");
        return lv_[level].comp ? lv_[level].comp->far_ranges() : 0;
    }
    int numa_node() const { return numa_node_; }
    size_t numa_cpus() const { return numa_cpus_.size(); }
    void bind_host_thread() const { pin_current_thread(numa_cpus_); }
    const std::vector<double>& placement_ms() const { return placement_.ms; }
    size_t placement_best() const { return placement_.kept; }
    const PlacementReport& placement() const { return placement_; }

  private:
    struct Pending
    {
        bool has = false;
        int kind = 0;
        uint32_t index = 0;
        bool scale = false;
    };

    void run_batch(const uint8_t* dsrc, uint32_t n);
    void place_level(StageLevel& L, uint8_t* at = nullptr);
    void place_rings_at(uint64_t offset);
    void calibrate_placement();
    void build_shard_order(StageLevel& L);
    void ensure_comp_slots(StageLevel& L);
    void compress_layer_host(StageLevel& L, uint32_t slot, uint64_t layer,
                             const Compression& c);
    FusedParams fused_params(const uint8_t* dsrc, uint32_t n, uint32_t n_fused,
                             uint32_t rh_log2, bool tail);
    void run_fused(const uint8_t* dsrc, uint32_t n);
    void run_fused3d(const uint8_t* dsrc, uint32_t n);
    void run_generic(const uint8_t* dsrc, uint32_t n);
    void enter_layers(StageLevel& L, uint64_t first_fid, uint64_t n);
    void enter_layer(StageLevel& L, uint64_t layer);
    LevelGeom geom(StageLevel& L, uint64_t fid0, bool tiles,
                   uint8_t* scratch) const;
    void tile_addr(const StageLevel& L, uint64_t fid, uint64_t* off,
                   uint32_t* flag_off, uint32_t* tag) const;
    const uint8_t* frame_ptr(uint32_t level, uint32_t index,
                             const uint8_t* dsrc) const;

    ArrayDesc desc_;
    StageOptions opt_;
    size_t bpp_;
    std::vector<StageLevel> lv_;
    bool fused_2d_ = true;
    bool fused_3d_ = false;
    uint32_t g3d_ = 1, zmask3d_ = 0;
    uint32_t n_fused_ = 0;
    uint32_t rh_log2_ = 4;
    uint64_t max_frames_ = 0;
    uint64_t slab_len_ = 0, slab_done_ = 0;
    std::vector<uint64_t> slab_skip_;
    hipStream_t own_stream_ = nullptr;
    hipStream_t stream_ = nullptr;
    PinnedBuf h_stage_[2];
    DevBuf d_stage_[2];
    hipEvent_t h2d_ev_[2] = { nullptr, nullptr };
    hipEvent_t consume_ev_[2] = { nullptr, nullptr };
    bool consume_rec_[2] = { false, false };
    int stage_idx_ = 0;
    hipStream_t h2d_ = nullptr, d2h_ = nullptr;
    hipStream_t comp_ = nullptr;
    hipStream_t comp_lo_ = nullptr;
    hipStream_t comp_lo2_ = nullptr;
    hipStream_t comp_stream(const StageLevel& L) const
    {
        const size_t k = size_t(&L - &lv_[0]);
        return k == 0 ? comp_ : k <= 2 ? comp_lo_ : comp_lo2_;
    }
    std::unique_ptr<CopyPool> pool_;
    std::unique_ptr<TaskPool> zpool_;
    std::unique_ptr<SplitPool> split_pool_;
    std::vector<int> numa_cpus_;
    int numa_node_ = -1;
    bool xy_ = false;
    bool xy_direct_ = false;
    bool xy_src_ = false;
    uint32_t acq_rows_ = 0, acq_cols_ = 0;
    DevBuf xbuf_;
    std::vector<std::pair<hipEvent_t, uint64_t>> inflight_;
    size_t inflight_head_ = 0;
    std::vector<hipEvent_t> free_ev_;
    uint64_t appended_ = 0, consumed_ = 0;
    struct Ticket
    {
        hipEvent_t ev = nullptr;
        hsa_signal_t sig{ 0 };
    };
    std::deque<Ticket> tickets_;
    uint64_t tickets_issued_ = 0, tickets_done_ = 0, last_ticket_ = 0;
    uint64_t issue_ticket();
    uint64_t issue_ticket(hsa_signal_t sig);
    bool sdma_d2h_ = false;
    hsa_agent_t hsa_gpu_{ 0 }, hsa_cpu_{ 0 };
    std::vector<hsa_signal_t> free_sig_;
    void note_consumed(hipStream_t s, uint64_t frames);
    void retire_consumed(bool wait);
    uint32_t nt_mode_ = 7;
    uint32_t knobs_ = 0;
    uint32_t xcd_rot_ = 0;
    std::vector<Pending> pend_;
    bool timing_ = false;
    std::vector<std::pair<hipEvent_t, hipEvent_t>> ev_pairs_;
    size_t ev_used_ = 0;
    double timed_ms_ = 0;
    uint64_t timed_launches_ = 0;
    hipEvent_t mark_ev_[2] = { nullptr, nullptr };
    hipEvent_t ext_ev_ = nullptr;
    PlacementReport placement_;
    std::vector<DevBuf> held_;
    DevBuf arena_;
    uint64_t arena_rings_ = 0;
    bool arena_fallback_ = false;
    std::mutex access_mu_;
    std::vector<int> granted_;
    void grant_access(int device);
    bool finalized_ = false;
};

const char* downsampling_method_name(int32_t method);
std::string downsampling_metadata_json(int32_t method);

class GpuDownsampler
{
  public:
    explicit GpuDownsampler(const ArrayDesc& desc);
    ~GpuDownsampler();

    uint32_t n_levels() const { return uint32_t(levels_.size()); }
    const std::vector<Dim>& level_dims(uint32_t level) const;
    void add_frame(const void* frame, size_t nbytes, int mem);
    bool take_frame(uint32_t level, void* dst, size_t cap, int mem,
                    size_t* nbytes);
    const char* method_name() const;
    std::string metadata_json() const;

  private:
    struct Lv
    {
        uint32_t W, H, planes;
        bool xy_shrinks;
        DevBuf cur, pending, partial;
        bool has_pending = false, has_partial = false;
        uint32_t count = 0;
    };
    int32_t dtype_, method_;
    size_t bpp_;
    std::vector<std::vector<Dim>> levels_;
    std::vector<Lv> lv_;
    DevBuf input_;
    DevBuf d_op_;
// ... 6 lines not shown
```

include/aqz_gpu.h:

```cpp
#ifndef AQZ_GPU_H
#define AQZ_GPU_H

#include <stddef.h>
#include <stdint.h>

#ifdef __cplusplus
extern "C" {
#endif

typedef int32_t aqz_status;
#define AQZ_STATUS_SUCCESS 0
#define AQZ_STATUS_INVALID_ARGUMENT 1
#define AQZ_STATUS_OVERFLOW 2
#define AQZ_STATUS_INVALID_INDEX 3
#define AQZ_STATUS_NOT_YET_IMPLEMENTED 4
#define AQZ_STATUS_INTERNAL_ERROR 5
#define AQZ_STATUS_OUT_OF_MEMORY 6
#define AQZ_STATUS_INVALID_SETTINGS 9
#define AQZ_STATUS_WRITE_OUT_OF_BOUNDS 12

enum
{
    AQZ_DTYPE_UINT8 = 0,
    AQZ_DTYPE_UINT16,
// ... 150 lines not shown
aqz_status aqz_stage_copy_layer(aqz_stage* st, uint32_t level, uint64_t layer,
                                void* dst, size_t cap, uint8_t* has_data,
                                size_t has_data_cap, int32_t mem);
aqz_status aqz_stage_copy_layer_async(aqz_stage* st, uint32_t level,
                                      uint64_t layer, void* dst, size_t cap,
                                      uint8_t* has_data, size_t has_data_cap);
aqz_status aqz_stage_wait_copies(aqz_stage* st);
uint64_t aqz_stage_last_ticket(const aqz_stage* st);
uint64_t aqz_stage_copies_completed(aqz_stage* st);
aqz_status aqz_stage_wait_ticket(aqz_stage* st, uint64_t ticket);

aqz_status aqz_stage_band_geometry(const aqz_stage* st, uint32_t level,
                                   int32_t* supported, uint32_t* n_bands,
                                   uint64_t* frames_per_band,
                                   uint32_t* chunks_per_band);
aqz_status aqz_stage_copy_band_async(aqz_stage* st, uint32_t level,
                                     uint64_t layer, uint32_t band, void* dst,
                                     size_t cap, uint8_t* has_data,
                                     size_t has_data_cap);

typedef struct
{
    uint64_t device_bytes;
    uint64_t pinned_bytes;
} aqz_memory_usage;
aqz_status aqz_stage_memory_usage(const aqz_stage* st, aqz_memory_usage* out);
aqz_status aqz_stage_estimate_memory(const aqz_array_desc* desc,
                                     const aqz_stage_options* opt,
                                     aqz_memory_usage* out);
aqz_status aqz_stage_bind_host_thread(const aqz_stage* st);
aqz_status aqz_host_alloc(size_t bytes, void** out);
void aqz_host_free(void* p);
aqz_status aqz_stage_device_layer(aqz_stage* st, uint32_t level,
                                  uint64_t layer, void** chunks,
                                  uint32_t** has_data);
#define AQZ_CODEC_NONE 0
#define AQZ_CODEC_BLOSC_LZ4 1
#define AQZ_CODEC_BLOSC_ZSTD 2
#define AQZ_CODEC_ZSTD 3
typedef struct
{
    int32_t codec;
    int32_t clevel;
    int32_t shuffle;
} aqz_compression;

aqz_status aqz_stage_compress_layer(aqz_stage* st, uint32_t level, uint64_t layer,
                                    const aqz_compression* comp);
aqz_status aqz_stage_compressed_offsets(aqz_stage* st, uint32_t level,
                                        uint64_t layer, uint64_t* offsets, size_t n);
aqz_status aqz_stage_copy_compressed_async(aqz_stage* st, uint32_t level,
                                           uint64_t layer, void* dst, size_t cap);
aqz_status aqz_stage_compression_done(aqz_stage* st, uint32_t level, uint64_t layer,
                                      int32_t* done);

typedef struct
{
    uint32_t chunk;
    uint32_t shard;
    uint32_t internal;
    uint32_t reserved;
    uint64_t offset;
    uint64_t nbytes;
} aqz_chunk_entry;
aqz_status aqz_stage_compressed_entries(aqz_stage* st, uint32_t level,
                                        uint64_t layer, aqz_chunk_entry* out,
                                        size_t n);
aqz_status aqz_stage_shard_geometry(const aqz_stage* st, uint32_t level,
                                    uint32_t* chunks_per_shard,
                                    uint32_t* number_of_shards,
                                    uint32_t* layers_per_shard);
size_t aqz_shard_table_bytes(uint32_t chunks_per_shard);
aqz_status aqz_shard_table(const uint64_t* offsets, const uint64_t* extents,
                           uint32_t chunks_per_shard, void* out, size_t cap);
uint32_t aqz_crc32c(const void* data, size_t n);

typedef struct aqz_compressor aqz_compressor;
aqz_status aqz_compressor_create(uint64_t chunk_bytes, uint32_t typesize,
                                 const aqz_compression* comp, aqz_compressor** out);
void aqz_compressor_destroy(aqz_compressor* c);
uint64_t aqz_compressor_max_bytes(uint64_t chunk_bytes, uint32_t n_chunks);
uint64_t aqz_compressor_scratch_bytes(const aqz_compression* comp, uint64_t chunk_bytes,
                                      uint32_t typesize, uint32_t n_chunks);
aqz_status aqz_compressor_run(aqz_compressor* c, const void* chunks, uint64_t pitch,
                              uint32_t n_chunks, void* dst, size_t dst_cap,
                              uint64_t* offsets, void* stream);
uint32_t aqz_compressor_blocksize(const aqz_compressor* c);

aqz_status aqz_stage_import_frames(aqz_stage* dst, aqz_stage* src, uint32_t level,
                                   uint64_t layer, uint32_t first, uint32_t count);

aqz_status aqz_stage_split_level0_host(aqz_stage* st, const void* frames, uint64_t n_frames,
                                       uint64_t first_frame, uint32_t chunk0, void* dst,
                                       size_t cap, uint8_t* has_data, size_t has_data_cap);
aqz_status aqz_stage_split_level0_rows(const aqz_stage* st, const void* frame,
                                       uint64_t frame_id, uint32_t row_begin,
                                       uint32_t row_end, void* frame_copy, uint32_t chunk0,
                                       void* dst, size_t cap, uint8_t* has_data,
                                       size_t has_data_cap);
aqz_status aqz_dims_split_frame_rows(const aqz_dims* d, const void* frame, uint64_t frame_id,
                                     uint32_t row_begin, uint32_t row_end, uint32_t chunk0,
                                     void* dst, size_t cap, uint8_t* has_data,
                                     size_t has_data_cap);

aqz_status aqz_stage_finalize(aqz_stage* st);

#define AQZ_DECODE_OK 0
#define AQZ_DECODE_SKIPPED 1
#define AQZ_DECODE_BAD_HEADER 2
#define AQZ_DECODE_CORRUPT 3
#define AQZ_DECODE_UNSUPPORTED 4
#define AQZ_DECODE_CODEC_LZ4 1u
#define AQZ_DECODE_CODEC_ZSTD 2u
#define AQZ_DECODE_ZSTD_PARALLEL 4u
typedef struct aqz_decompressor aqz_decompressor;
aqz_status aqz_decompressor_create(uint64_t max_chunk_bytes, uint32_t max_chunks,
                                   aqz_decompressor** out);
aqz_status aqz_decompressor_create_for(uint64_t max_chunk_bytes, uint32_t max_chunks,
                                       uint32_t codecs, aqz_decompressor** out);
void aqz_decompressor_destroy(aqz_decompressor* d);
uint64_t aqz_decompressor_scratch_bytes(uint64_t max_chunk_bytes, uint32_t max_chunks);
uint64_t aqz_decompressor_scratch_bytes_for(uint64_t max_chunk_bytes, uint32_t max_chunks,
                                            uint32_t codecs);
aqz_status aqz_decompressor_run(aqz_decompressor* d, const void* frames, size_t frames_bytes,
                                const uint64_t* offsets, uint32_t n_chunks, void* dst,
                                uint64_t pitch, uint64_t chunk_bytes, uint32_t* status,
                                void* stream);

aqz_status aqz_stage_verify_layer(aqz_stage* st, uint32_t level, uint64_t layer,
                                  const void* frames, size_t frames_bytes);
aqz_status aqz_stage_verify_prepare(aqz_stage* st, uint32_t codecs);
aqz_status aqz_stage_verify_result(aqz_stage* st, uint32_t level, uint64_t layer,
                                   uint32_t* n_bad, uint32_t* first_bad);

aqz_status aqz_shard_table_parse(const void* table, size_t nbytes, uint32_t chunks_per_shard,
                                 uint64_t* offsets, uint64_t* extents, int32_t* crc_ok);

typedef struct aqz_reader aqz_reader;
typedef struct
{
    const aqz_dimension* dimensions;
    size_t dimension_count;
    int32_t data_type;
    const size_t* storage_dimension_order;
    uint32_t codecs;
    uint64_t max_frames_bytes;
    int32_t device;
} aqz_reader_desc;
aqz_status aqz_reader_create(const aqz_reader_desc* desc, aqz_reader** out);
void aqz_reader_destroy(aqz_reader* r);
uint64_t aqz_reader_device_bytes(const aqz_reader_desc* desc);
aqz_status aqz_reader_layout(const aqz_reader* r, aqz_level_layout* out);

aqz_status aqz_reader_load_frames(aqz_reader* r, const void* frames, size_t frames_bytes,
                                  int32_t mem, const uint64_t* offsets,
                                  const uint32_t* chunk_of_frame, uint32_t n_frames,
                                  int32_t codec, void* stream);
aqz_status aqz_reader_load_chunks(aqz_reader* r, const void* chunks, uint64_t pitch,
                                  const uint32_t* has_data, uint32_t tag, void* stream);
aqz_status aqz_reader_read_frames(aqz_reader* r, uint32_t first, uint32_t count, void* dst,
                                  uint64_t dst_stride, void* stream);
aqz_status aqz_reader_status(aqz_reader* r, uint32_t* status, size_t cap, uint32_t* n_bad);

#ifdef __cplusplus
}
#endif
// ... 2 lines not shown
```

include/aqz_gpu_bench.h:

```cpp
#ifndef AQZ_GPU_BENCH_H
#define AQZ_GPU_BENCH_H

#include "aqz_gpu.h"

#ifdef __cplusplus
extern "C" {
#endif

typedef struct
{
    uint32_t force_levels;
    int32_t skip_level0_split;
    uint32_t placement_tries;
    uint32_t placement_reps;
    uint32_t placement_flags;
    uint32_t knobs;
    uint32_t nt_policy;
    uint32_t xcd_rot;
    uint32_t region_rows_log2;
    uint32_t zstd_flags;
    uint32_t ring_malloc_flags;
    uint64_t chunk_pad_bytes;
    uint64_t ring_spacer_bytes;
    uint64_t ring_arena_bytes;
} aqz_stage_bench_options;

aqz_status aqz_stage_estimate_memory_bench(const aqz_array_desc* desc,
                                           const aqz_stage_options* opt,
                                           const aqz_stage_bench_options* bench,
                                           aqz_memory_usage* out);

typedef struct
{
    uint32_t n;
    uint32_t kept;
    uint32_t reps;
    uint32_t mode;
    double ms[32];
    double kept_ms_final;
    uint64_t peak_device_bytes;
    double probe_bus_gbs;
    double expected_ms;
    uint64_t alg_bytes;
    uint32_t accepted;
    uint32_t stop;
    double probe_gbs[32];
} aqz_placement_report;
aqz_status aqz_stage_placement_report(const aqz_stage* st, aqz_placement_report* out);

aqz_status aqz_stage_create_bench(const aqz_array_desc* desc,
                                  const aqz_stage_options* opt,
                                  const aqz_stage_bench_options* bench,
                                  aqz_stage** out);

aqz_status aqz_stage_set_tuning(aqz_stage* st, uint32_t knobs, uint32_t nt);

aqz_status aqz_stage_bench_replace_rings(aqz_stage* st, uint32_t level_mask);

aqz_status aqz_stage_bench_set_ring_offset(aqz_stage* st, uint64_t offset);

aqz_status aqz_stage_enable_kernel_timing(aqz_stage* st, int32_t enable);
aqz_status aqz_stage_kernel_timing(aqz_stage* st, double* total_ms,
                                   uint64_t* launches);
aqz_status aqz_stage_timing_mark(aqz_stage* st, int32_t which);
aqz_status aqz_stage_timing_elapsed(aqz_stage* st, double* ms);
const char* aqz_stage_dominant_kernel(const aqz_stage* st);
uint32_t aqz_stage_zstd_far_ranges(const aqz_stage* st, uint32_t level);

aqz_status aqz_stage_placement(const aqz_stage* st, double* ms, size_t cap,
                               size_t* n, uint32_t* kept);

aqz_status aqz_stage_host_affinity(const aqz_stage* st, int32_t* numa_node,
                                   uint32_t* n_cpus);

enum
{
    AQZ_PROBE_READ = 0,
    AQZ_PROBE_COPY = 1,
    AQZ_PROBE_COPY_THIRD = 2,
    AQZ_PROBE_READ_THIRD = 3,
    AQZ_PROBE_PLAIN_STORES = 0x100,
    AQZ_PROBE_PIECES = 0x200,
    AQZ_PROBE_DEEP = 0x400
};
aqz_status aqz_probe_hbm(int32_t device, int32_t shape, uint64_t bytes, uint32_t reps,
                         double* ms, uint64_t* read_bytes);

typedef struct
{
    uint32_t zstd_parallel_frames;
    uint32_t zstd_serial_frames;
    uint32_t zstd_blocks;
    uint32_t zstd_sequences;
} aqz_decode_counts;
aqz_status aqz_decompressor_last_run_counts(aqz_decompressor* d, aqz_decode_counts* out);

#ifdef __cplusplus
}
#endif
#endif
```

integration/aqz_handoff.hh:

```
#pragma once

#include "aqz_gpu.h"

#include <algorithm>
#include <atomic>
#include <chrono>
#include <condition_variable>
#include <cstdlib>
#include <cstring>
#include <deque>
#include <functional>
#include <memory>
#include <mutex>
#include <string>
#include <thread>
#include <vector>

namespace aqz_binding {

class Lease
{
  public:
    Lease() = default;
    explicit Lease(std::atomic<int>* pins)
// ... 277 lines not shown
    }
    return p;
}

inline uint32_t
slabs_from_env()
{
    const char* e = std::getenv("AQZ_Z_SLABS");
    const int n = e ? std::atoi(e) : 1;
    return n > 1 ? uint32_t(n) : 1u;
}

struct MemoryEstimate
{
    uint64_t host_bytes = 0, device_bytes = 0;
};

inline aqz_status
estimate_memory(const aqz_array_desc& desc, const aqz_stage_options& opt,
                const HandoffOptions& o, uint32_t n_stages, MemoryEstimate* out)
{
    if (!out || n_stages == 0)
        return AQZ_STATUS_INVALID_ARGUMENT;
    *out = MemoryEstimate{};
    aqz_memory_usage st{};
    aqz_status s = aqz_stage_estimate_memory(&desc, &opt, &st);
    if (s != AQZ_STATUS_SUCCESS)
        return s;
    aqz_dims* base = nullptr;
    s = aqz_dims_create(desc.dimensions, desc.dimension_count, desc.data_type,
                        desc.storage_dimension_order, &base);
    if (s != AQZ_STATUS_SUCCESS)
        return s;
    std::vector<aqz_dimension> d0(aqz_dims_ndims(base));
    for (size_t i = 0; i < d0.size(); ++i)
        (void)aqz_dims_get(base, i, &d0[i]);
    aqz_dims_destroy(base);
    uint32_t nl = 0;
    s = aqz_pyramid_levels(d0.data(), d0.size(), desc.max_levels, &nl, nullptr, 0);
    std::vector<aqz_dimension> lv(size_t(nl) * d0.size());
    if (s == AQZ_STATUS_SUCCESS)
        s = aqz_pyramid_levels(d0.data(), d0.size(), desc.max_levels, &nl, lv.data(),
                               lv.size());
    if (s != AQZ_STATUS_SUCCESS)
        return s;
    const size_t nd = d0.size();
    static const size_t bpp_of[] = { 1, 2, 4, 8, 1, 2, 4, 8, 4, 8 };
    const size_t bpp = desc.data_type >= 0 && desc.data_type < 10 ? bpp_of[desc.data_type] : 8;
    const uint64_t fb = uint64_t(d0[nd - 1].array_size_px) * d0[nd - 2].array_size_px * bpp;
    const uint32_t batch = std::max<uint32_t>(1, o.batch_frames);
    const uint32_t B = opt.max_batch_frames ? opt.max_batch_frames : 64;
    const uint32_t slots = std::max<uint32_t>(1, o.host_slots);
    const bool compressed = o.comp.codec != AQZ_CODEC_NONE;
    const char* hz = std::getenv("AQZ_ZSTD_HOST");
    const bool host_zstd = hz && std::atoi(hz) != 0 &&
                           (o.comp.codec == AQZ_CODEC_BLOSC_ZSTD || o.comp.codec == AQZ_CODEC_ZSTD);
    uint64_t host = uint64_t(n_stages) * (2 * uint64_t(batch) * fb + st.pinned_bytes);
    uint64_t dev = uint64_t(n_stages) * st.device_bytes;
    for (uint32_t l = 0; l < nl; ++l) {
        aqz_dims* d = nullptr;
        s = aqz_dims_create(&lv[size_t(l) * nd], nd, desc.data_type, nullptr, &d);
        if (s != AQZ_STATUS_SUCCESS)
            return s;
        const uint64_t bpc = aqz_dims_bytes_per_chunk(d);
        const uint32_t n_chunks = aqz_dims_number_of_chunks_in_memory(d);
        const uint64_t F = std::max<uint64_t>(1, aqz_dims_frames_per_chunk_layer(d));
        int32_t banded = 0;
        uint32_t n_bands = 1, per_band = n_chunks;
        uint64_t fpb = 0;
        (void)aqz_dims_dim1_banding(d, &banded, &n_bands, &fpb, &per_band);
        aqz_dims_destroy(d);
        if (compressed || !banded)
            per_band = n_chunks;
        const uint64_t cap =
          compressed ? aqz_compressor_max_bytes(bpc, n_chunks) : bpc * per_band;
        host += uint64_t(slots) * (cap + per_band);
        if (!compressed)
            continue;
        const uint64_t ring_slots =
          std::max<uint64_t>(opt.layer_slots ? opt.layer_slots : 2, (B - 1 + F - 1) / F + 1);
        const uint64_t offs = (uint64_t(n_chunks) + 1) * 8;
        uint64_t ldev = ring_slots * (aqz_compressor_max_bytes(bpc, n_chunks) + offs) +
                        aqz_compressor_scratch_bytes(&o.comp, bpc, uint32_t(bpp), n_chunks);
        uint64_t lhost = ring_slots * offs;
        if (host_zstd) {
            ldev += bpc * n_chunks;
            lhost += ring_slots * (bpc * n_chunks + n_chunks);
        }
        dev += uint64_t(n_stages) * ldev;
        host += uint64_t(n_stages) * lhost;
    }
    out->host_bytes = host;
    out->device_bytes = dev;
    return AQZ_STATUS_SUCCESS;
}

class Handoff
{
  public:
    Handoff(std::vector<aqz_stage*> stages, const SlabPlan& plan, uint64_t frame_bytes,
            const HandoffOptions& o, HandoffSink& sink)
      : st_(std::move(stages))
      , plan_(plan)
      , frame_bytes_(frame_bytes)
      , opt_(o)
      , sink_(sink)
    {
        opt_.batch_frames = std::max<uint32_t>(1, opt_.batch_frames);
        opt_.host_slots = std::max<uint32_t>(1, opt_.host_slots);
        if (st_.empty() || (st_.size() > 1 && plan_.begin.size() != st_.size())) {
            status_ = AQZ_STATUS_INVALID_ARGUMENT;
            return;
        }
        in_.resize(st_.size());
        for (Input& in : in_)
            for (int j = 0; j < 2; ++j)
                status_ =
                  worse(status_, aqz_host_alloc(size_t(opt_.batch_frames) * frame_bytes_,
                                                reinterpret_cast<void**>(&in.buf[j])));
        aqz_stage* st0 = st_[0];
        const uint32_t nl = aqz_stage_n_levels(st0);
        levels_.resize(nl);
        for (uint32_t l = 0; l < nl && status_ == AQZ_STATUS_SUCCESS; ++l) {
            Level& L = levels_[l];
            status_ = worse(status_, aqz_stage_level_layout(st0, l, &L.lay));
            int32_t banded = 0;
            status_ = worse(status_, aqz_stage_band_geometry(st0, l, &banded, &L.n_bands,
                                                             &L.frames_per_band,
                                                             &L.chunks_per_band));
            L.compressed = opt_.comp.codec != AQZ_CODEC_NONE;
            L.host = l == 0 && opt_.level0_on_host;
            if (L.host && L.compressed)
                status_ = worse(status_, AQZ_STATUS_INVALID_ARGUMENT);
            if (L.compressed || !banded) {
                L.n_bands = 1;
                L.frames_per_band = L.lay.frames_per_layer;
                L.chunks_per_band = L.lay.chunks_per_layer;
            }
            if (st_.size() > 1) {
                aqz_dimension d[16];
                size_t nd = 0;
                status_ = worse(status_, aqz_stage_level_dims(st0, l, d, 16, &nd));
                L.planes = nd >= 3 ? d[nd - 3].array_size_px : 0;
                if (L.planes == 0 || plan_.planes % L.planes != 0)
                    status_ = worse(status_, AQZ_STATUS_INVALID_SETTINGS);
            }
            const size_t cap =
              L.compressed ? size_t(aqz_compressor_max_bytes(L.lay.bytes_per_chunk,
                                                            L.lay.chunks_per_layer))
                           : size_t(L.lay.bytes_per_chunk) * L.chunks_per_band;
            for (uint32_t i = 0; i < opt_.host_slots; ++i) {
                auto s = std::make_unique<Slot>();
                s->cap = cap;
                status_ = worse(status_, aqz_host_alloc(cap, reinterpret_cast<void**>(&s->buf)));
                status_ = worse(status_, aqz_host_alloc(L.chunks_per_band,
                                                        reinterpret_cast<void**>(&s->has)));
                if (L.host && s->buf)
                    std::memset(s->buf, 0, cap);
                s->ent.resize(L.chunks_per_band);
                L.slots.push_back(std::move(s));
            }
            if (L.host) {
                L.ragged_last_band =
                  L.n_bands > 1 &&
                  L.lay.frames_per_layer - uint64_t(L.n_bands - 1) * L.frames_per_band <
                    L.frames_per_band;
// ... 679 lines not shown
```

Before: 2621.

## Run zstd far-match kernel ahead on dedicated per-level streams

Adds a per-level compression stream plan that gives deeper pyramid levels their own low-priority streams and optionally a separate far stream. The zstd far-match kernel runs on that far stream as soon as the level's ring slot is ready, double-buffering its scratch so the next layer's far pass can overlap the current parse. The aim is to overlap compression work across levels and layers instead of serializing it on shared streams. The cost is extra device memory for the second far buffer, more events and streams, and extra synchronization. The benchmarked path is uncompressed device-resident downsampling, so it may not touch this code.

```diff
diff --git a/acquire-zarr_amd/aqz/__init__.py b/acquire-zarr_amd/aqz/__init__.py
--- a/acquire-zarr_amd/aqz/__init__.py
+++ b/acquire-zarr_amd/aqz/__init__.py
@@ -246,6 +246,9 @@
         "aqz_stage_timing_elapsed": ([vp, C.POINTER(C.c_double)], i32),
         "aqz_stage_dominant_kernel": ([vp], C.c_char_p),
         "aqz_stage_zstd_far_ranges": ([vp, u32], u32),
+        "aqz_stage_compression_streams": ([vp, C.POINTER(u32), C.POINTER(u32), u32], i32),
+        "aqz_stage_compressor_extra_bytes": ([C.POINTER(CompressionC), u64, u32, u32, u32, u32],
+                                             u64),
         "aqz_probe_hbm": ([i32, i32, u64, u32, C.POINTER(C.c_double), C.POINTER(u64)], i32),
         "aqz_stage_placement": ([vp, C.POINTER(C.c_double), sz, C.POINTER(sz),
                                  C.POINTER(u32)], i32),
@@ -463,6 +466,12 @@
     return lib().aqz_compressor_scratch_bytes(C.byref(c), chunk_bytes, typesize, n_chunks)
 
 
+def stage_compressor_extra_bytes(codec, chunk_bytes, typesize, n_chunks, n_levels, level):
+    c = CompressionC(*codec)
+    return lib().aqz_stage_compressor_extra_bytes(C.byref(c), chunk_bytes, typesize, n_chunks,
+                                                  n_levels, level)
+
+
 def pyramid_levels(dims, max_levels=0):
     d = _dims_c(dims)
     n = C.c_uint32(0)
@@ -772,6 +781,13 @@
     def zstd_far_ranges(self, level):
         return lib().aqz_stage_zstd_far_ranges(self.h, level)
 
+    def compression_streams(self):
+        n = self.n_levels()
+        comp, far = (C.c_uint32 * n)(), (C.c_uint32 * n)()
+        _check(lib().aqz_stage_compression_streams(self.h, comp, far, n),
+               "compression_streams")
+        return list(comp), [None if f == 0xffffffff else f for f in far]
+
     def bind_host_thread(self):
         _check(lib().aqz_stage_bind_host_thread(self.h), "bind_host_thread")
 
diff --git a/acquire-zarr_amd/csrc/aqz_capi.cpp b/acquire-zarr_amd/csrc/aqz_capi.cpp
--- a/acquire-zarr_amd/csrc/aqz_capi.cpp
+++ b/acquire-zarr_amd/csrc/aqz_capi.cpp
@@ -991,6 +991,26 @@
 }
 
 aqz_status
+aqz_stage_compression_streams(const aqz_stage* st, uint32_t* per_level, uint32_t* far_per_level,
+                              uint32_t n)
+{
+    if (!st || !st->st)
+        return AQZ_STATUS_INVALID_ARGUMENT;
+    return guard([&] {
+        const std::vector<uint32_t>& comp = st->st->level_comp_streams();
+        const std::vector<uint32_t> far = st->st->level_far_streams();
+        if (n > comp.size())
+            throw Error(3, "more levels than the stage has");
+        for (uint32_t k = 0; k < n; ++k) {
+            if (per_level)
+                per_level[k] = comp[k];
+            if (far_per_level)
+                far_per_level[k] = far[k];
+        }
+    });
+}
+
+aqz_status
 aqz_stage_host_affinity(const aqz_stage* st, int32_t* numa_node, uint32_t* n_cpus)
 {
     if (!st)
@@ -1125,6 +1145,23 @@
     return s == AQZ_STATUS_SUCCESS ? n : 0;
 }
 
+uint64_t
+aqz_stage_compressor_extra_bytes(const aqz_compression* comp, uint64_t chunk_bytes,
+                                 uint32_t typesize, uint32_t n_chunks, uint32_t n_levels,
+                                 uint32_t level)
+{
+    if (!comp || level >= n_levels)
+        return 0;
+    uint64_t n = 0;
+    const aqz_status s = guard([&] {
+        const Compression c = to_compression(comp);
+        Compressor check(chunk_bytes, typesize, c);
+        if (comp_stream_plan(n_levels).far[level] != kNoStream)
+            n = Compressor::far_ahead_bytes(c, chunk_bytes, typesize, n_chunks);
+    });
+    return s == AQZ_STATUS_SUCCESS ? n : 0;
+}
+
 uint32_t
 aqz_compressor_blocksize(const aqz_compressor* c)
 {
diff --git a/acquire-zarr_amd/csrc/aqz_codec.hh b/acquire-zarr_amd/csrc/aqz_codec.hh
--- a/acquire-zarr_amd/csrc/aqz_codec.hh
+++ b/acquire-zarr_amd/csrc/aqz_codec.hh
@@ -185,4 +185,14 @@
 
 hipError_t launch_zstd(const ZstdParams& p, hipStream_t stream);
 
+struct ZstdFarAhead
+{
+    hipStream_t stream;
+    hipEvent_t ready;
+    hipEvent_t buf_free;
+    hipEvent_t done;
+    hipEvent_t parsed;
+};
+hipError_t launch_zstd(const ZstdParams& p, hipStream_t stream, const ZstdFarAhead* far);
+
 }
diff --git a/acquire-zarr_amd/csrc/aqz_codec.hip b/acquire-zarr_amd/csrc/aqz_codec.hip
--- a/acquire-zarr_amd/csrc/aqz_codec.hip
+++ b/acquire-zarr_amd/csrc/aqz_codec.hip
@@ -2163,6 +2163,12 @@
 hipError_t
 launch_zstd(const ZstdParams& p, hipStream_t stream)
 {
+    return launch_zstd(p, stream, nullptr);
+}
+
+hipError_t
+launch_zstd(const ZstdParams& p, hipStream_t stream, const ZstdFarAhead* fa)
+{
     if (p.n_chunks == 0)
         return hipSuccess;
     const uint64_t nseg = uint64_t(p.n_chunks) * p.nseg;
@@ -2197,8 +2203,19 @@
                 const uint32_t R = p.far_ranges;
                 if (!(R == 1 || R == 2 || R == 4 || R == 8))
                     return hipErrorInvalidValue;
+                const hipStream_t fs = fa ? fa->stream : stream;
+                if (fa) {
+                    for (hipEvent_t w : { fa->ready, fa->buf_free })
+                        if (w && (e = hipStreamWaitEvent(fs, w, 0)) != hipSuccess)
+                            return e;
+                }
                 hipLaunchKernelGGL(zstd_far, dim3(uint32_t(nseg * p.far_slices * R)),
-                                   dim3(kFarThreads), size_t(4) << p.far_log, stream, p);
+                                   dim3(kFarThreads), size_t(4) << p.far_log, fs, p);
+                if (fa) {
+                    if ((e = hipEventRecord(fa->done, fs)) != hipSuccess ||
+                        (e = hipStreamWaitEvent(stream, fa->done, 0)) != hipSuccess)
+                        return e;
+                }
             }
             if (p.phist == 0 && !p.far)
                 hipLaunchKernelGGL((zstd_parse<0, kLz4HashLog>), gd, dim3(64), 0, stream, p);
@@ -2212,6 +2229,8 @@
                 hipLaunchKernelGGL((zstd_parse<kZHist1, 13, true>), gd, dim3(64), 0, stream, p);
             else
                 hipLaunchKernelGGL((zstd_parse<kZHist2, 14, true>), gd, dim3(64), 0, stream, p);
+            if (fa && p.far && (e = hipEventRecord(fa->parsed, stream)) != hipSuccess)
+                return e;
         } else {
             hipLaunchKernelGGL(zstd_hist, dim3(uint32_t(nblk)), dim3(256), 0, stream, p);
         }
diff --git a/acquire-zarr_amd/csrc/aqz_engine.cpp b/acquire-zarr_amd/csrc/aqz_engine.cpp
--- a/acquire-zarr_amd/csrc/aqz_engine.cpp
+++ b/acquire-zarr_amd/csrc/aqz_engine.cpp
@@ -305,6 +305,26 @@
     return true;
 }
 
+CompStreamPlan
+comp_stream_plan(uint32_t n_levels)
+{
+    CompStreamPlan pl;
+    pl.comp.assign(n_levels, 0);
+    pl.far.assign(n_levels, kNoStream);
+    const uint32_t deep = n_levels > 2 ? n_levels - 2 : 0;
+    const uint32_t n_least = std::min(deep, kHwQueues - 1);
+    pl.three.assign(n_levels, 0);
+    for (uint32_t k = 1; k < n_levels; ++k) {
+        pl.comp[k] = k == 1 ? 1 : 2 + std::min(k - 2, n_least - 1);
+        pl.three[k] = k <= 2 ? 1 : 2;
+    }
+    uint32_t next = 2 + n_least;
+    for (uint32_t k = 0; k < n_levels && next - 2 < kHwQueues; ++k)
+        pl.far[k] = next++;
+    pl.n_streams = std::max(next, 2u);
+    return pl;
+}
+
 Stage::Stage(const ArrayDesc& desc, const StageOptions& opt)
   : desc_(desc)
   , opt_(opt)
@@ -536,8 +556,17 @@
                   "hipStreamCreate");
         for (hipStream_t* cs : { &comp_, &comp_lo_ })
             hip_check(hipStreamCreateWithFlags(cs, hipStreamNonBlocking), "hipStreamCreate");
-        hip_check(hipStreamCreateWithPriority(&comp_lo2_, hipStreamNonBlocking, least),
-                  "hipStreamCreate");
+        const CompStreamPlan plan = comp_stream_plan(uint32_t(lv_.size()));
+        level_own_ = plan.comp;
+        level_three_ = plan.three;
+        level_comp_ = plan.three;
+        level_far_ = plan.far;
+        comp_streams_.assign(plan.n_streams, nullptr);
+        comp_streams_[0] = comp_;
+        comp_streams_[1] = comp_lo_;
+        for (uint32_t i = 2; i < plan.n_streams; ++i)
+            hip_check(hipStreamCreateWithPriority(&comp_streams_[i], hipStreamNonBlocking, least),
+                      "hipStreamCreate");
     }
     if (const char* e = std::getenv("AQZ_D2H_SDMA"); e && std::atoi(e) != 0)
         sdma_d2h_ = find_hsa_agents(desc.device, &hsa_gpu_, &hsa_cpu_);
@@ -549,6 +578,7 @@
         L.ready_ev.assign(L.n_slots, nullptr);
         L.copy_ev.assign(L.n_slots, nullptr);
         L.copy_pending.assign(L.n_slots, 0);
+        L.peer_ev.resize(L.n_slots);
         for (uint32_t s = 0; s < L.n_slots; ++s) {
             hip_check(hipEventCreateWithFlags(&L.ready_ev[s], hipEventDisableTiming),
                       "hipEventCreate");
@@ -842,13 +872,26 @@
 Stage::~Stage()
 {
     zpool_.reset();
-    for (auto& L : lv_)
-        for (auto& v : L.peer_ev)
-            for (const auto& e : v)
-                (void)hipEventSynchronize(e.get());
+    {
+        std::lock_guard<std::mutex> lk(access_mu_);
+        for (auto& L : lv_)
+            for (auto& v : L.peer_ev)
+                for (const auto& e : v)
+                    (void)hipEventSynchronize(e.get());
+    }
     if (stream_)
         (void)hipStreamSynchronize(stream_);
-    for (hipStream_t s : { h2d_, comp_, comp_lo_, comp_lo2_, d2h_ })
+    for (hipStream_t s : comp_streams_)
+        if (s)
+            (void)hipStreamSynchronize(s);
+    for (auto& L : lv_)
+        L.comp.reset();
+    std::vector<hipStream_t> streams = comp_streams_;
+    if (streams.empty())
+        streams = { comp_, comp_lo_ };
+    streams.push_back(h2d_);
+    streams.push_back(d2h_);
+    for (hipStream_t s : streams)
         if (s) {
             (void)hipStreamSynchronize(s);
             (void)hipStreamDestroy(s);
@@ -950,9 +993,8 @@
 {
     hip_check(hipStreamSynchronize(h2d_), "hipStreamSynchronize");
     hip_check(hipStreamSynchronize(stream_), "hipStreamSynchronize");
-    hip_check(hipStreamSynchronize(comp_), "hipStreamSynchronize");
-    hip_check(hipStreamSynchronize(comp_lo_), "hipStreamSynchronize");
-    hip_check(hipStreamSynchronize(comp_lo2_), "hipStreamSynchronize");
+    for (hipStream_t s : comp_streams_)
+        hip_check(hipStreamSynchronize(s), "hipStreamSynchronize");
     hip_check(hipStreamSynchronize(d2h_), "hipStreamSynchronize");
     retire_consumed(true);
 }
@@ -1090,9 +1132,8 @@
 void
 Stage::wait_copies()
 {
-    hip_check(hipStreamSynchronize(comp_), "hipStreamSynchronize");
-    hip_check(hipStreamSynchronize(comp_lo_), "hipStreamSynchronize");
-    hip_check(hipStreamSynchronize(comp_lo2_), "hipStreamSynchronize");
+    for (hipStream_t s : comp_streams_)
+        hip_check(hipStreamSynchronize(s), "hipStreamSynchronize");
     hip_check(hipStreamSynchronize(d2h_), "hipStreamSynchronize");
     (void)copies_completed(true);
 }
@@ -2019,10 +2060,45 @@
     return 0u;
 }
 
+Compressor::~Compressor()
+{
+    for (hipEvent_t e : { far_done_ev_, parsed_ev_[0], parsed_ev_[1] })
+        if (e)
+            (void)hipEventDestroy(e);
+}
+
+static bool
+far_ahead_settings(const Compression& c, uint32_t typesize)
+{
+    return c.codec == 3 && zstd_far_slices(c, typesize) != 0;
+}
+
+void
+Compressor::set_far_stream(hipStream_t s)
+{
+    far_stream_ = nullptr;
+    if (!s || !far_ahead_settings(c_, typesize_))
+        return;
+    for (hipEvent_t* e : { &far_done_ev_, &parsed_ev_[0], &parsed_ev_[1] })
+        if (!*e)
+            hip_check(hipEventCreateWithFlags(e, hipEventDisableTiming), "hipEventCreate");
+    far_stream_ = s;
+}
+
+uint64_t
+Compressor::far_ahead_bytes(const Compression& c, uint64_t chunk_bytes, uint32_t typesize,
+                            uint32_t n_chunks)
+{
+    return far_ahead_settings(c, typesize) ? uint64_t(n_chunks) * chunk_bytes * 4 : 0;
+}
+
 uint64_t
 Compressor::scratch_bytes(const Compression& c, uint64_t chunk_bytes, uint32_t typesize,
-                          uint32_t n_chunks)
-{
+                          uint32_t n_chunks, bool far_stream)
+{
+    if (far_stream)
+        return scratch_bytes(c, chunk_bytes, typesize, n_chunks) +
+               far_ahead_bytes(c, chunk_bytes, typesize, n_chunks);
     const uint64_t n = n_chunks;
     const bool store_only = c.codec != 3 && c.clevel == 0;
     uint64_t b = n * 4 + n + n * 8;
@@ -2060,10 +2136,10 @@
 void
 Compressor::run(const uint8_t* chunks, uint64_t pitch, uint32_t n_chunks,
                 const uint32_t* flags, uint32_t tag, uint8_t* out, uint64_t* offsets,
-                hipStream_t stream, const uint32_t* order)
+                hipStream_t stream, const uint32_t* order, hipEvent_t ready)
 {
     if (c_.codec != 1) {
-        run_zstd(chunks, pitch, n_chunks, flags, tag, out, offsets, stream, order);
+        run_zstd(chunks, pitch, n_chunks, flags, tag, out, offsets, stream, order, ready);
         return;
     }
     const uint64_t ns = uint64_t(n_chunks) * g_.spc;
@@ -2096,9 +2172,10 @@
 void
 Compressor::run_zstd(const uint8_t* chunks, uint64_t pitch, uint32_t n_chunks,
                      const uint32_t* flags, uint32_t tag, uint8_t* out, uint64_t* offsets,
-                     hipStream_t stream, const uint32_t* order)
+                     hipStream_t stream, const uint32_t* order, hipEvent_t ready)
 {
     const bool blosc = c_.codec == 2;
+    ZstdFarAhead fa{};
     ZstdParams p{};
     p.chunks = chunks;
     p.pitch = pitch;
@@ -2156,8 +2233,25 @@
                    (p.src_pitch & 3u) == 0 && (p.seg_bytes & 3u) == 0;
         far = far && tune_.far != 0;
         if (far) {
-            alloc_large(far_, nseg * p.seg_bytes * 4, tune_.vmm);
-            p.far = reinterpret_cast<uint32_t*>(far_.p);
+            const bool ahead = far_stream_ && ready && p.src == chunks;
+            const uint32_t fb = ahead ? uint32_t(ahead_runs_ & 1u) : 0u;
+            DevBuf& fbuf = fb ? far2_ : far_;
+            const uint64_t fbytes = nseg * p.seg_bytes * 4;
+            if (far_stream_ && fbuf.p && fbuf.n < fbytes) {
+                hip_check(hipStreamSynchronize(far_stream_), "hipStreamSynchronize");
+                hip_check(hipStreamSynchronize(stream), "hipStreamSynchronize");
+            }
+            alloc_large(fbuf, fbytes, tune_.vmm);
+            p.far = reinterpret_cast<uint32_t*>(fbuf.p);
+            if (ahead) {
+                fa.stream = far_stream_;
+                fa.ready = ready;
+                fa.buf_free = parsed_rec_[fb] ? parsed_ev_[fb] : nullptr;
+                fa.done = far_done_ev_;
+                fa.parsed = parsed_ev_[fb];
+                parsed_rec_[fb] = true;
+                ++ahead_runs_;
+            }
             p.phist = 0;
             const uint64_t wgs = nseg * p.far_slices;
             const uint64_t steps = (uint64_t(p.seg_bytes) + kZSub - 1) / kZSub;
@@ -2231,7 +2325,7 @@
     p.offsets = offsets;
     p.cstart = reinterpret_cast<uint64_t*>(cstart_.p);
     p.out = out;
-    hip_check(launch_zstd(p, stream), "zstd launch");
+    hip_check(launch_zstd(p, stream, fa.stream ? &fa : nullptr), "zstd launch");
 }
 
 void
@@ -2364,7 +2458,8 @@
     if (level >= lv_.size())
         throw Error(3, "level out of range");
     StageLevel& L = lv_[level];
-    const hipStream_t cs = comp_stream(L);
+    hipStream_t cs = comp_stream(L);
+    const hipStream_t fs = far_stream(L);
     if (!L.ring.p)
         throw Error(1, "level 0 is not split on the device by this stage");
     const uint32_t slot = uint32_t(layer % L.n_slots);
@@ -2377,10 +2472,17 @@
     if (!L.comp || L.comp_cfg.codec != c.codec || L.comp_cfg.clevel != c.clevel ||
         L.comp_cfg.shuffle != c.shuffle) {
         hip_check(hipStreamSynchronize(cs), "hipStreamSynchronize");
+        if (fs)
+            hip_check(hipStreamSynchronize(fs), "hipStreamSynchronize");
         hip_check(hipStreamSynchronize(d2h_), "hipStreamSynchronize");
         L.comp = std::make_unique<Compressor>(L.bpc, uint32_t(bpp_), c, opt_.codec);
         L.comp->set_plane_bytes(uint64_t(L.tw) * L.th * bpp_);
+        L.comp->set_far_stream(fs);
         L.comp_cfg = c;
+        level_comp_[level] = Compressor::far_ahead_bytes(c, L.bpc, uint32_t(bpp_), 1) != 0
+                               ? level_own_[level]
+                               : level_three_[level];
+        cs = comp_stream(L);
     }
     ensure_comp_slots(L);
     if (L.zjob[slot])
@@ -2406,7 +2508,7 @@
                 reinterpret_cast<const uint32_t*>(L.flags.p) + size_t(slot) * L.n_chunks,
                 uint32_t(layer / L.n_slots + 1), L.cframes[slot].p,
                 reinterpret_cast<uint64_t*>(L.coffsets[slot].p), cs,
-                reinterpret_cast<const uint32_t*>(L.shard_order.p));
+                reinterpret_cast<const uint32_t*>(L.shard_order.p), L.ready_ev[slot]);
     hip_check(hipMemcpyAsync(L.h_coffsets[slot].p, L.coffsets[slot].p,
                              (size_t(L.n_chunks) + 1) * 8, hipMemcpyDeviceToHost, cs),
               "hipMemcpyAsync");
@@ -2798,8 +2900,6 @@
         std::shared_ptr<ihipEvent_t> ev(e, [](hipEvent_t x) { (void)hipEventDestroy(x); });
         hip_check(hipEventRecord(e, stream_), "hipEventRecord");
         std::lock_guard<std::mutex> lk(src->access_mu_);
-        if (S->peer_ev.empty())
-            S->peer_ev.resize(S->n_slots);
         S->peer_ev[slot].push_back(std::move(ev));
     }
 }
diff --git a/acquire-zarr_amd/csrc/aqz_engine.hh b/acquire-zarr_amd/csrc/aqz_engine.hh
--- a/acquire-zarr_amd/csrc/aqz_engine.hh
+++ b/acquire-zarr_amd/csrc/aqz_engine.hh
@@ -119,7 +119,14 @@
     }
     void run(const uint8_t* chunks, uint64_t pitch, uint32_t n_chunks,
              const uint32_t* flags, uint32_t tag, uint8_t* out, uint64_t* offsets,
-             hipStream_t stream, const uint32_t* order = nullptr);
+             hipStream_t stream, const uint32_t* order = nullptr, hipEvent_t ready = nullptr);
+    ~Compressor();
+    Compressor(const Compressor&) = delete;
+    Compressor& operator=(const Compressor&) = delete;
+    void set_far_stream(hipStream_t s);
+    bool far_ahead() const { return far_stream_ != nullptr; }
+    static uint64_t far_ahead_bytes(const Compression& c, uint64_t chunk_bytes,
+                                    uint32_t typesize, uint32_t n_chunks);
     const BloscGeom& geom() const { return g_; }
     void set_plane_bytes(uint64_t b) { plane_bytes_ = b; }
     uint64_t chunk_bytes() const { return nbytes_; }
@@ -133,10 +140,11 @@
         return 0;
     }
     static uint64_t scratch_bytes(const Compression& c, uint64_t chunk_bytes,
-                                  uint32_t typesize, uint32_t n_chunks);
+                                  uint32_t typesize, uint32_t n_chunks,
+                                  bool far_stream = false);
     uint64_t device_bytes() const
     {
-        uint64_t n = scratch_.n + ssize_.n + spos_.n + fsize_.n + mode_.n + cstart_.n;
+        uint64_t n = scratch_.n + ssize_.n + spos_.n + fsize_.n + mode_.n + cstart_.n + far2_.n;
         for (const DevBuf* b : { &zin_, &hist_, &scount_, &bkind_, &bpay_, &bpos_, &tab_, &carrier_,
                                  &sraw_, &lits_, &seqs_, &snseq_, &snlit_, &stail_, &bltype_,
                                  &bnseq_, &sqt_, &scarrier_, &sval_,
@@ -148,7 +156,13 @@
   private:
     void run_zstd(const uint8_t* chunks, uint64_t pitch, uint32_t n_chunks,
                   const uint32_t* flags, uint32_t tag, uint8_t* out, uint64_t* offsets,
-                  hipStream_t stream, const uint32_t* order);
+                  hipStream_t stream, const uint32_t* order, hipEvent_t ready);
+    hipStream_t far_stream_ = nullptr;
+    hipEvent_t far_done_ev_ = nullptr;
+    hipEvent_t parsed_ev_[2] = { nullptr, nullptr };
+    bool parsed_rec_[2] = { false, false };
+    uint64_t ahead_runs_ = 0;
+    DevBuf far2_;
     Compression c_;
     CodecTuning tune_;
     uint64_t nbytes_ = 0;
@@ -334,6 +348,15 @@
 bool shard_major_order(const ArrayDimensions& ad, std::vector<uint32_t>& order,
                        std::vector<uint32_t>& shard, std::vector<uint32_t>& internal0);
 
+constexpr uint32_t kHwQueues = 4;
+constexpr uint32_t kNoStream = 0xffffffffu;
+struct CompStreamPlan
+{
+    std::vector<uint32_t> comp, far, three;
+    uint32_t n_streams = 0;
+};
+CompStreamPlan comp_stream_plan(uint32_t n_levels);
+
 class Stage
 {
   public:
@@ -399,6 +422,15 @@
             throw Error(3, "level out of range");
         return lv_[level].comp ? lv_[level].comp->far_ranges() : 0;
     }
+    const std::vector<uint32_t>& level_comp_streams() const { return level_comp_; }
+    std::vector<uint32_t> level_far_streams() const
+    {
+        std::vector<uint32_t> v(lv_.size(), kNoStream);
+        for (size_t k = 0; k < lv_.size(); ++k)
+            if (lv_[k].comp && lv_[k].comp->far_ahead())
+                v[k] = level_far_[k];
+        return v;
+    }
     int numa_node() const { return numa_node_; }
     size_t numa_cpus() const { return numa_cpus_.size(); }
     void bind_host_thread() const { pin_current_thread(numa_cpus_); }
@@ -460,11 +492,16 @@
     hipStream_t h2d_ = nullptr, d2h_ = nullptr;
     hipStream_t comp_ = nullptr;
     hipStream_t comp_lo_ = nullptr;
-    hipStream_t comp_lo2_ = nullptr;
+    std::vector<hipStream_t> comp_streams_;
+    std::vector<uint32_t> level_comp_, level_far_, level_own_, level_three_;
     hipStream_t comp_stream(const StageLevel& L) const
     {
-        const size_t k = size_t(&L - &lv_[0]);
-        return k == 0 ? comp_ : k <= 2 ? comp_lo_ : comp_lo2_;
+        return comp_streams_[level_comp_[size_t(&L - &lv_[0])]];
+    }
+    hipStream_t far_stream(const StageLevel& L) const
+    {
+        const uint32_t i = level_far_[size_t(&L - &lv_[0])];
+        return i == kNoStream ? nullptr : comp_streams_[i];
     }
     std::unique_ptr<CopyPool> pool_;
     std::unique_ptr<TaskPool> zpool_;
diff --git a/include/aqz_gpu.h b/include/aqz_gpu.h
--- a/include/aqz_gpu.h
+++ b/include/aqz_gpu.h
@@ -256,6 +256,9 @@
 uint64_t aqz_compressor_max_bytes(uint64_t chunk_bytes, uint32_t n_chunks);
 uint64_t aqz_compressor_scratch_bytes(const aqz_compression* comp, uint64_t chunk_bytes,
                                       uint32_t typesize, uint32_t n_chunks);
+uint64_t aqz_stage_compressor_extra_bytes(const aqz_compression* comp, uint64_t chunk_bytes,
+                                          uint32_t typesize, uint32_t n_chunks,
+                                          uint32_t n_levels, uint32_t level);
 aqz_status aqz_compressor_run(aqz_compressor* c, const void* chunks, uint64_t pitch,
                               uint32_t n_chunks, void* dst, size_t dst_cap,
                               uint64_t* offsets, void* stream);
diff --git a/include/aqz_gpu_bench.h b/include/aqz_gpu_bench.h
--- a/include/aqz_gpu_bench.h
+++ b/include/aqz_gpu_bench.h
@@ -66,6 +66,8 @@
 aqz_status aqz_stage_timing_elapsed(aqz_stage* st, double* ms);
 const char* aqz_stage_dominant_kernel(const aqz_stage* st);
 uint32_t aqz_stage_zstd_far_ranges(const aqz_stage* st, uint32_t level);
+aqz_status aqz_stage_compression_streams(const aqz_stage* st, uint32_t* per_level,
+                                         uint32_t* far_per_level, uint32_t n);
 
 aqz_status aqz_stage_placement(const aqz_stage* st, double* ms, size_t cap,
                                size_t* n, uint32_t* kept);
diff --git a/integration/aqz_handoff.hh b/integration/aqz_handoff.hh
--- a/integration/aqz_handoff.hh
+++ b/integration/aqz_handoff.hh
@@ -383,6 +383,7 @@
         const uint64_t offs = (uint64_t(n_chunks) + 1) * 8;
         uint64_t ldev = ring_slots * (aqz_compressor_max_bytes(bpc, n_chunks) + offs) +
                         aqz_compressor_scratch_bytes(&o.comp, bpc, uint32_t(bpp), n_chunks);
+        ldev += aqz_stage_compressor_extra_bytes(&o.comp, bpc, uint32_t(bpp), n_chunks, nl, l);
         uint64_t lhost = ring_slots * offs;
         if (host_zstd) {
             ldev += bpc * n_chunks;
```

Result: slower. 2508 (-4.3%).
